# isabella232/kyverno

Hardware: AMD Instinct MI355X
Metric: resource×rule validate evals/sec (node) (higher is better)
Workload: dtype u8; 1 GPU; C2: synthetic Pods x 100 validate.pattern rules (image globs, ?*, quantities, |-lists); rules=100, pairs_per_gpu=100000000, output=full, parallelism=resource-shard x1, engine=specialized

## Files before the change

kyverno_amd/csrc/kvapi.cpp:

```cpp
#include <hip/hip_runtime.h>
#include <rccl/rccl.h>

#include <chrono>
#include <cstdio>
#include <cstring>

#define KVRT_DEVICE 1
#include "kvrt.hpp"
#include "kvdev.h"

namespace kvh {

struct DevPolicySet {
  DevBuf prog, preds, alts, conjs, atoms, rules, filters, kinds, strrefs, strpairs, sels, sellabels, selexprs, kgs,
      gsegs, gwords, pstr, fword, fbit, flist, frule, rcompact, gsdesc, gsmem;
  DevBuf view_dev;
  uint32_t gs_groups = 0, gs_members = 0;
  DevPS view{};
  std::vector<hipModule_t> mods;
  std::vector<hipFunction_t> fns;
  std::map<uint32_t, std::vector<hipFunction_t>> vfns;
  const std::vector<hipFunction_t>& fns_for(uint32_t full) const {
    auto it = vfns.find(full);
    return it == vfns.end() ? fns : it->second;
// ... 16 lines not shown
      }
    }
  }
};

struct DevBatchRes {
  DevBuf nodes, vals, res, kvs, bstr, nsbits, koff, klen, kstr, nsms, lsets, asets, tuprep, tupkent, kentrep, view_dev;
  DevBuf dpreds, dalts, dconjs, datoms, dgsegs, dgwords, dpstr, dps, dleaf, dynst;
  DevBuf pcol, pcold, pfam, perow;
  double pcol_ms = 0;
  DevBuf pre[5], dn[7], feg[2], fed[7], fe[5], fep[3], feacc, ferec, prest, dnst;
  double pre_ms = 0, deny_ms = 0, fe_ms = 0;
  DevBatch view{};
};
}

kv_policyset::kv_policyset() = default;
kv_policyset::~kv_policyset() = default;

namespace {

DevPolicySet& dev_ps(kv_policyset* s, int device) {
  std::lock_guard<std::mutex> g(s->mu);
  auto it = s->dev.find(device);
  if (it != s->dev.end()) return *it->second;
  auto d = std::make_unique<DevPolicySet>();
  const PolicySet& ps = s->ps;
  d->prog.upload(ps.prog, device);
  d->preds.upload(ps.preds, device);
  d->alts.upload(ps.alts, device);
  d->conjs.upload(ps.conjs, device);
  d->atoms.upload(ps.atoms, device);
  d->rules.upload(ps.rules, device);
  d->filters.upload(ps.filters, device);
  d->kinds.upload(ps.kinds, device);
  d->strrefs.upload(ps.strrefs, device);
  d->strpairs.upload(ps.strpairs, device);
  d->sels.upload(ps.selectors, device);
  d->sellabels.upload(ps.sellabels, device);
  d->selexprs.upload(ps.selexprs, device);
  d->kgs.upload(ps.kg_specs, device);
  d->gsegs.upload(ps.gsegs, device);
  d->gwords.upload(ps.gwords, device);
  d->pstr.upload_raw(ps.strs.data(), ps.strs.size(), device);
  DevPS& v = d->view;
  v.prog = (const Inst*)d->prog.p;
  v.preds = (const Pred*)d->preds.p;
  v.alts = (const Alt*)d->alts.p;
  v.conjs = (const Conj*)d->conjs.p;
  v.atoms = (const Atom*)d->atoms.p;
  v.rules = (const RuleRec*)d->rules.p;
  v.filters = (const MFilter*)d->filters.p;
  v.kinds = (const KindSpec*)d->kinds.p;
  v.strrefs = (const StrRef*)d->strrefs.p;
  v.strpairs = (const StrPair*)d->strpairs.p;
  v.sels = (const Selector*)d->sels.p;
  v.sellabels = (const SelLabel*)d->sellabels.p;
  v.selexprs = (const SelExpr*)d->selexprs.p;
  v.kg_specs = (const uint32_t*)d->kgs.p;
  v.gsegs = (const GSeg*)d->gsegs.p;
  v.gwords = (const GWord*)d->gwords.p;
  v.n_rules = (uint32_t)ps.rules.size();
  v.n_filters = (uint32_t)ps.filters.size();
  v.n_sels = (uint32_t)ps.selectors.size();
  v.pstr = (const uint8_t*)d->pstr.p;
  v.star_id = ps.lookup("*");
  if (v.star_id == KEY_NONE) v.star_id = KEY_NONE - 1;
  d->dev = device;
  if (s->jit) {
    const JitImage& J = *s->jit;
    std::map<std::string, hipFunction_t> byname;
    for (size_t i = 0; i < J.codes.size(); i++) {
      hipModule_t m;
      HIPCHK(hipModuleLoadData(&m, J.codes[i].data()));
      d->mods.push_back(m);
      hipFunction_t f;
      HIPCHK(hipModuleGetFunction(&f, m, J.kernel_name[i].c_str()));
      byname[J.kernel_name[i]] = f;
    }
    for (const JitImage::Variant& v : J.variants) {
      std::map<std::string, hipFunction_t> vname;
      for (size_t i = 0; i < v.codes.size() && i < J.kernel_name.size(); i++) {
        if (v.codes[i].empty()) continue;
        hipModule_t m;
        HIPCHK(hipModuleLoadData(&m, v.codes[i].data()));
        d->mods.push_back(m);
        hipFunction_t f;
        HIPCHK(hipModuleGetFunction(&f, m, J.kernel_name[i].c_str()));
        vname[J.kernel_name[i]] = f;
      }
      std::vector<hipFunction_t>& fv = d->vfns[v.full];
      for (auto& ch : J.chunks) {
        auto it = vname.find(ch.name);
        fv.push_back(it != vname.end() ? it->second : byname.at(ch.name));
      }
    }
    for (auto& ch : J.chunks) {
      auto it = byname.find(ch.name);
      if (it == byname.end()) throw std::runtime_error("specialized kernel " + ch.name + " missing");
      hipFunction_t f = it->second;
      d->fns.push_back(f);
      if (getenv("KVGPU_VERBOSE")) {
        int regs = 0, local = 0;
        (void)hipFuncGetAttribute(&regs, HIP_FUNC_ATTRIBUTE_NUM_REGS, f);
        (void)hipFuncGetAttribute(&local, HIP_FUNC_ATTRIBUTE_LOCAL_SIZE_BYTES, f);
        fprintf(stderr, "[kvgpu] %s: %zu rules, %d VGPRs, %d B scratch/lane\n", ch.name.c_str(), ch.rules.size(), regs,
                local);
      }
    }
    d->rcompact.upload(J.rec_compact, device);
    if (!J.gs_desc.empty()) {
      d->gs_groups = (uint32_t)(J.gs_desc.size() / 4u);
      d->gs_members = J.gs_members;
      d->gsdesc.upload(J.gs_desc, device);
      d->gsmem.upload(J.gs_mem, device);
    }
    if (J.mtup_words) {
      d->mtup_words = J.mtup_words;
      d->fac_slots = J.fac_slots;
      d->fword.upload(J.fac_word, device);
      d->fbit.upload(J.fac_bit, device);
      d->flist.upload(J.fac_flist, device);
      d->frule.upload(J.fac_rule, device);
      v.fac_word = (const uint32_t*)d->fword.p;
      v.fac_bit = (const uint32_t*)d->fbit.p;
      v.fac_flist = (const uint32_t*)d->flist.p;
      v.fac_rule = (const uint32_t*)d->frule.p;
      v.fac_slots = J.fac_slots;
      v.fac_words = J.mtup_words;
    }
    if (J.memo_words) {
      d->ptab_fn = byname.at("kvj_ptab");
      d->memo_words = J.memo_words;
      d->ptab_rows = (uint32_t)((J.memo_preds.size() + J.ptab_row - 1) / J.ptab_row);
    }
  }
  if (!ps.fpats.empty()) d->view_dev.upload_raw(&d->view, sizeof(DevPS), device);
  auto& ref = *d;
  s->dev[device] = std::move(d);
  return ref;
}

void build_pcol(const JitImage& J, const Batch& b, DevBatchRes* d, int device) {
  const auto t0 = std::chrono::steady_clock::now();
  const uint32_t nf = (uint32_t)J.fam_ncols.size(), j0 = J.fam_ncols.at(0);
  const uint64_t groups64 = (b.res.size() + KV_WG - 1) / KV_WG * (KV_WG / KV_LANES);
  if (groups64 > 0x3FFFFFFull) throw std::runtime_error("path columns: too many resources");
  const uint32_t groups = (uint32_t)groups64;
  d->pcold.upload(J.cols, device);
  d->perow.alloc((size_t)std::max<uint32_t>(1u, nf - 1) * (groups + 1) * sizeof(uint32_t), device);
  HIPCHK(hipMemset(d->perow.p, 0, d->perow.n));
  std::vector<ColFam> fams(nf);
  uint32_t n_wide = 0, n_narrow = 0;
  for (uint32_t f = 0; f < nf; f++) {
    fams[f].arr_col = J.fam_arr[f];
    fams[f].ncols = J.fam_ncols[f];
    fams[f].nw = J.fam_nw.at(f);
    fams[f].nb = J.fam_nb.at(f);
    fams[f].nn = J.fam_nn.at(f);
    fams[f].erow = f ? (uint32_t*)d->perow.p + (size_t)(f - 1) * (groups + 1) : nullptr;
    n_wide += fams[f].nw;
    n_narrow += fams[f].nn;
  }
  if (n_narrow && b.vals.size() + KV_PTAB_PSEUDO >= (1ull << KV_COL_PAYLOAD))
    throw std::runtime_error("path columns: more than 2^28 distinct values");
  d->pfam.upload(fams, device);
  const DevBatch* Bd = (const DevBatch*)d->view_dev.p;
  const ColDesc* cd = (const ColDesc*)d->pcold.p;
  std::vector<uint32_t> erow;
  if (nf > 1) {
    HIPCHK(launch_pcol_rows(Bd, cd, (const ColFam*)d->pfam.p, nf, groups, nullptr));
    erow.resize((size_t)(nf - 1) * (groups + 1));
    HIPCHK(hipMemcpy(erow.data(), d->perow.p, erow.size() * sizeof(uint32_t), hipMemcpyDeviceToHost));
  }
  auto row_words = [&](uint32_t f) { return (uint64_t)(3u * fams[f].nw + fams[f].nb + fams[f].nn) * KV_LANES; };
  const uint64_t root_words = (uint64_t)groups * row_words(0);
  uint64_t words = root_words;
  for (uint32_t f = 1; f < nf; f++) {
    fams[f].off_lo = (uint32_t)words;
    fams[f].off_hi = (uint32_t)(words >> 32);
    words += (uint64_t)erow[(size_t)(f - 1) * (groups + 1) + groups] * row_words(f);
  }
  if (words >= (1ull << 32)) throw std::runtime_error("path columns: more than 2^32 words");
  HIPCHK(hipMemcpy(d->pfam.p, fams.data(), fams.size() * sizeof(ColFam), hipMemcpyHostToDevice));
  d->pcol.alloc(std::max<uint64_t>(words, 1) * sizeof(uint32_t), device);
  uint32_t* pool = (uint32_t*)d->pcol.p;
  if (words > root_words) HIPCHK(hipMemset(pool + root_words, 0, (words - root_words) * sizeof(uint32_t)));
  HIPCHK(launch_pcol_build(Bd, cd, (const ColFam*)d->pfam.p, 0, j0, groups, false, pool, nullptr));
  HIPCHK(launch_pcol_build(Bd, cd, (const ColFam*)d->pfam.p, j0, (uint32_t)J.cols.size() - j0, groups, true, pool,
                           nullptr));
  HIPCHK(hipStreamSynchronize(nullptr));
  d->view.pcol = pool;
  d->pcol_ms = std::chrono::duration<double, std::milli>(std::chrono::steady_clock::now() - t0).count();
  if (getenv("KVGPU_VERBOSE"))
    fprintf(stderr,
            "[kvgpu] path columns: %u wide + %u narrow columns in %u families, %llu bytes (%.1f per resource), built in "
            "%.2f ms\n",
            n_wide, n_narrow, nf, (unsigned long long)(words * sizeof(uint32_t)),
            b.res.empty() ? 0.0 : (double)(words * sizeof(uint32_t)) / (double)b.res.size(), d->pcol_ms);
}

std::shared_ptr<DevBatchRes> dev_batch(kv_batch* bt, const PolicySet& ps, int device, const DevPS* pdev) {
  std::lock_guard<std::mutex> g(bt->mu);
  auto it = bt->dev.find(device);
  if (it != bt->dev.end()) return it->second;
  auto d = std::make_shared<DevBatchRes>();
  const Batch& b = bt->b;
  if (b.rmask.size() != b.n_rows || b.rwide.size() != b.n_rows || b.roff.size() != b.n_rows)
    throw std::runtime_error("batch: packed row arrays do not match the row count");
  hipStream_t us = StreamPool::get().take(device, hipStreamNonBlocking);
  DevBuf pc, rm, rw, ro;
  pc.upload_async(b.tcells, device, us);
  rm.upload_async(b.rmask, device, us);
  rw.upload_async(b.rwide, device, us);
  ro.upload_async(b.roff, device, us);
  d->vals.upload_async(b.vals, device, us);
  d->nodes.alloc(b.n_cells() * sizeof(Node), device);
  HIPCHK(launch_expand_rows((const uint64_t*)pc.p, (const uint64_t*)rm.p, (const uint64_t*)rw.p, (const uint32_t*)ro.p,
                            (const Val*)d->vals.p, b.n_rows, (Node*)d->nodes.p, us));
  d->res.upload_async(b.res, device, us);
  d->kvs.upload(b.kvs, device);
  d->bstr.upload_raw(b.strs.data(), b.strs.size(), device);
  d->nsbits.upload(b.ns_bits, device);
  std::vector<uint32_t> off, len;
  std::string ks;
  key_table(ps, b, &off, &len, &ks);
  d->koff.upload(off, device);
  d->klen.upload(len, device);
  d->kstr.upload_raw(ks.data(), ks.size(), device);
  d->nsms.upload(b.nsms, device);
  d->lsets.upload(b.lsets, device);
  d->asets.upload(b.asets, device);
  d->tuprep.upload(b.tup_rep, device);
  d->tupkent.upload(b.tup_kent, device);
  d->kentrep.upload(b.kent_rep, device);
  DevBatch& v = d->view;
  v.nodes = (const Node*)d->nodes.p;
  v.vals = (const Val*)d->vals.p;
  v.res = (const Res*)d->res.p;
  v.kvs = (const KV*)d->kvs.p;
  v.bstr = (const uint8_t*)d->bstr.p;
  v.ns_bits = (const uint32_t*)d->nsbits.p;
  v.key_off = (const uint32_t*)d->koff.p;
  v.key_len = (const uint32_t*)d->klen.p;
  v.kstr = (const uint8_t*)d->kstr.p;
  v.nsms = (const StrRef*)d->nsms.p;
  v.lsets = (const KVSet*)d->lsets.p;
  v.asets = (const KVSet*)d->asets.p;
  v.n_nsm = (uint32_t)b.nsms.size();
  v.n_lsets = (uint32_t)b.lsets.size();
  v.n_asets = (uint32_t)b.asets.size();
  v.ns_words = b.ns_words;
  v.n_res = (uint32_t)b.res.size();
  v.tup_rep = (const uint32_t*)d->tuprep.p;
  v.n_tup = (uint32_t)b.tup_rep.size();
  v.tup_kent = (const uint32_t*)d->tupkent.p;
  v.kent_rep = (const uint32_t*)d->kentrep.p;
  v.n_kent = (uint32_t)b.kent_rep.size();
  v.n_ns = (uint32_t)b.namespaces.size();
  {
    const DynHost& h = bt->dyn_host(ps);
    d->dpreds.upload(h.tbl.preds, device);
    d->dalts.upload(h.tbl.alts, device);
    d->dconjs.upload(h.tbl.conjs, device);
    d->datoms.upload(h.tbl.atoms, device);
    d->dgsegs.upload(h.tbl.gsegs, device);
    d->dgwords.upload(h.tbl.gwords, device);
    d->dpstr.upload_raw(h.tbl.strs.data(), h.tbl.strs.size(), device);
    DevPS dv{};
    dv.preds = (const Pred*)d->dpreds.p;
    dv.alts = (const Alt*)d->dalts.p;
    dv.conjs = (const Conj*)d->dconjs.p;
    dv.atoms = (const Atom*)d->datoms.p;
    dv.gsegs = (const GSeg*)d->dgsegs.p;
    dv.gwords = (const GWord*)d->dgwords.p;
    dv.pstr = (const uint8_t*)d->dpstr.p;
    d->dps.upload_raw(&dv, sizeof(DevPS), device);
    d->dleaf.upload(h.dleaf, device);
    d->dynst.upload(h.dyn_st, device);
    v.dps = (const DevPS*)d->dps.p;
    v.dleaf = (const uint32_t*)d->dleaf.p;
    v.dyn_st = (const uint8_t*)d->dynst.p;
  }
  auto up = [&](DevBuf* bufs, std::initializer_list<const std::vector<uint32_t>*> src, const uint32_t** dp) {
    for (const std::vector<uint32_t>* v : src) {
      bufs->alloc(std::max<size_t>(v->size() * sizeof(uint32_t), 16), device);
      if (!v->empty()) HIPCHK(hipMemcpyAsync(bufs->p, v->data(), v->size() * sizeof(uint32_t), hipMemcpyHostToDevice, us));
      *dp++ = (const uint32_t*)(bufs++)->p;
    }
  };
  auto up_blocks = [&](DevBuf* bufs, const CondHost& h, bool strict) {
    const uint32_t* dp[7] = {};
    up(bufs, {&h.sets, &h.ents, &h.outc, &h.truth, &h.unk}, dp);
    if (strict) up(bufs + 5, {&h.err, &h.oos}, dp + 5);
    return CondBlocks{dp[0], dp[1], dp[2], dp[3], dp[4], dp[5], dp[6], h.words};
  };
  struct Timed {
    hipEvent_t e0, e1;
    double* ms;
  };
  std::vector<Timed> timed;
  auto timed_launch = [&](double* ms, auto&& launch) {
    Timed t{nullptr, nullptr, ms};
    HIPCHK(hipEventCreate(&t.e0));
    HIPCHK(hipEventCreate(&t.e1));
    HIPCHK(hipEventRecord(t.e0, us));
    HIPCHK(launch());
    HIPCHK(hipEventRecord(t.e1, us));
    timed.push_back(t);
  };
  CondHost pre, dn;
  FeHost fh;
  CondBlocks pt{}, dt{};
  FeTables ft{};
  FePatTables qt{};
  DevBuf erec;
  const uint32_t n_sets = (uint32_t)ps.csets.size(), n_dsets = (uint32_t)ps.dsets.size(),
                 n_fsets = (uint32_t)ps.fsets.size(), n_pats = (uint32_t)ps.fpats.size();
  if (n_sets && !b.res.empty()) {
    build_pre(ps, b, &pre);
    pt = up_blocks(d->pre, pre, false);
    d->prest.alloc((size_t)n_sets * b.res.size(), device);
    v.pre_st = (const uint8_t*)d->prest.p;
  }
  if (n_dsets && !b.res.empty()) {
    build_deny(ps, b, &dn);
    dt = up_blocks(d->dn, dn, true);
  }
  if (n_fsets && !b.res.empty()) {
    build_foreach(ps, b, &fh);
    const uint32_t *dp[5], *gp[2];
    up(d->fe, {&fh.sets, &fh.lists}, dp);
    up(d->feg, {&fh.gate.sets, &fh.gate.ents}, gp);
    ft = fh.view();
    ft.gate = ft.deny = up_blocks(d->fed, fh.deny, true);
    ft.gate.sets = gp[0]; ft.gate.ents = gp[1];
    up(d->fe + 2, {&fh.el_res, &fh.el_ord, &fh.lstate}, dp + 2);
    ft.sets = dp[0]; ft.lists = dp[1]; ft.el_res = dp[2]; ft.el_ord = dp[3]; ft.lstate = dp[4];
    d->feacc.alloc((size_t)n_fsets * b.res.size() * sizeof(uint32_t), device);
    if (n_pats) {
      const uint32_t* qp[3];
      up(d->fep, {&fh.pats, &fh.chain, &fh.first}, qp);
      qt = FePatTables{qp[0], qp[1], qp[2], n_pats};
// ... 1276 lines not shown
```

kyverno_amd/csrc/kvcol.h:

```cpp
#pragma once

KV_FN Node col_step(const Node* __restrict__ N, const Node& n, uint32_t step, uint32_t* idx) {
  const Node z{0u, 0u, 0u, 0u};
  if (*idx == ABSENT || node_type(n.kt) != NT_MAP) {
    *idx = ABSENT;
    return z;
  }
  if (step & KV_COL_SCAN) {
    const uint32_t key = step & ~KV_COL_SCAN;
    for (uint32_t q = 0; q < n.b; q++) {
      const uint32_t c = ni(n.a + q);
      const Node t = N[c];
      if (node_key(t.kt) == key) {
        *idx = c;
        return t;
      }
    }
    *idx = ABSENT;
    return z;
  }
  if (step >= n.b) {
    *idx = ABSENT;
    return z;
  }
  const uint32_t c = ni(n.a + step);
  const Node t = N[c];
  if (node_type(t.kt) == NT_ABSENT) {
    *idx = ABSENT;
    return z;
  }
  *idx = c;
  return t;
}

KV_FN Node col_walk(const Node* __restrict__ N, uint32_t idx, const ColDesc& d, uint32_t* out) {
  Node n{0u, 0u, 0u, 0u};
  if (idx != ABSENT) n = N[idx];
  for (uint32_t s = 0; s < d.nsteps && s < KV_COL_MAXD; s++) n = col_step(N, n, d.steps[s], &idx);
  *out = idx;
  return n;
}

KV_FN Node col_cell(const Node& n, uint32_t idx, uint32_t arr_c) {
  if (idx == ABSENT) return Node{0u, 0u, 0u, 0u};
  const uint32_t t = node_type(n.kt);
  return Node{t | KV_COL_PRESENT, n.a, n.b, t == NT_MAP ? idx : t == NT_ARR ? arr_c : n.c};
}

KV_FN uint64_t col_fam_off(const ColFam& F) { return (uint64_t)F.off_lo | (uint64_t)F.off_hi << 32; }
KV_FN uint32_t col_row_words(const ColFam& F) { return (3u * F.nw + F.nb + F.nn) * KV_LANES; }

KV_FN void col_put(uint32_t* __restrict__ pool, uint64_t row, const ColFam& F, const ColDesc& d, uint32_t lane,
                   const Node& n, uint32_t idx) {
  if (d.fmt == KV_COLF_NARROW) {
    pool[row + (size_t)(3u * F.nw + F.nb + d.pos) * KV_LANES + lane] = kv_narrow_cell(n.kt, n.a, idx);
    return;
  }
  uint32_t* __restrict__ w = pool + row + (size_t)d.pos * (3u * KV_LANES) + 3u * lane;
  w[0] = n.kt;
  w[1] = n.a;
  w[2] = n.c;
  if (d.fmt == KV_COLF_WIDEB) pool[row + (size_t)(3u * F.nw + d.bpos) * KV_LANES + lane] = n.b;
}
KV_FN Node col_get(const uint32_t* __restrict__ pool, uint64_t row, const ColFam& F, const ColDesc& d, uint32_t lane) {
  const uint32_t* __restrict__ w = pool + row + (size_t)d.pos * (3u * KV_LANES) + 3u * lane;
  return Node{w[0], w[1], pool[row + (size_t)(3u * F.nw + d.bpos) * KV_LANES + lane], w[2]};
}

KV_FN uint32_t col_rows(const DevBatch& B, const ColDesc* cols, const ColFam* fams, uint32_t f, uint32_t r) {
  if (r >= B.n_res) return 0u;
  uint32_t idx;
  const Node n = col_walk(B.nodes, ni(B.res[r].root), cols[fams[f].arr_col], &idx);
  return idx != ABSENT && node_type(n.kt) == NT_ARR ? n.b : 0u;
}

KV_FN void col_build_root(const DevBatch& B, const ColDesc* cols, const ColFam* fams, uint32_t c, uint32_t r,
                          uint32_t* __restrict__ pool) {
  const ColDesc& d = cols[c];
  Node cell{0u, 0u, 0u, 0u};
  uint32_t idx = ABSENT;
  if (r < B.n_res) {
    const Node n = col_walk(B.nodes, ni(B.res[r].root), d, &idx);
    uint32_t arr_c = 0u;
    if (d.arr_fam) {
      const ColFam& F = fams[d.arr_fam];
      arr_c = (uint32_t)(col_fam_off(F) + (uint64_t)F.erow[r >> 6] * col_row_words(F));
    }
    cell = col_cell(n, idx, arr_c);
  }
  col_put(pool, (uint64_t)(r >> 6) * col_row_words(fams[0]), fams[0], d, r & (KV_LANES - 1), cell, idx);
}

KV_FN void col_build_elem(const DevBatch& B, const ColDesc* cols, const ColFam* fams, uint32_t c, uint32_t r,
                          uint32_t* __restrict__ pool) {
  const ColDesc& d = cols[c];
  const ColFam& F = fams[d.fam];
  const uint32_t lane = r & (KV_LANES - 1);
  const Node a = col_get(pool, (uint64_t)(r >> 6) * col_row_words(fams[0]), fams[0], cols[F.arr_col], lane);
  if (node_type(a.kt) != NT_ARR || a.kt == 0u) return;
  for (uint32_t i = 0; i < a.b; i++) {
    uint32_t idx;
    const Node n = col_walk(B.nodes, ni(a.a + i), d, &idx);
    col_put(pool, (uint64_t)a.c + (uint64_t)i * col_row_words(F), F, d, lane, col_cell(n, idx, 0u), idx);
  }
}
```

kyverno_amd/csrc/kvdev.h:

```cpp
#pragma once
#include <hip/hip_runtime.h>
#include <stdint.h>

#include "kvcell.h"
#include "kv_layout.h"
#include "kvdevtypes.h"

namespace kv {

hipError_t launch_validate(const DevPS* P, const DevBatch* B, uint32_t n_res, const DevOut& O, uint32_t rule_begin,
                           uint32_t rule_end, hipStream_t stream);

struct CondBlocks;
hipError_t launch_cond(bool strict, const CondBlocks& T, uint32_t n_res, uint32_t n_sets, uint8_t* st, hipStream_t stream);

struct FeTables;
struct FePatTables;
hipError_t launch_foreach(const FeTables& T, uint32_t n_res, uint32_t* fe_acc, uint8_t* fe_st, hipStream_t stream,
                          const FePatTables* Q = nullptr, const DevPS* P = nullptr, const DevBatch* B = nullptr,
                          uint2* erec = nullptr, uint2* fe_rec = nullptr);

hipError_t launch_mtab(const DevPS* P, const DevBatch* B, uint32_t words, uint32_t max_entities, uint32_t* ns,
                       uint32_t* an, uint32_t* sl, hipStream_t stream);

hipError_t launch_mfac(const DevPS* P, const DevBatch* B, uint32_t slots, uint32_t max_entities, uint32_t words,
                       uint32_t n_tup, uint32_t* mtup, hipStream_t stream);

hipError_t launch_gather_rows(const uint8_t* in, const uint32_t* inv, uint64_t n_rules, uint64_t n_res, uint8_t* out,
                              hipStream_t stream);

hipError_t launch_remap_u32(uint32_t* a, uint64_t n, const uint32_t* map, hipStream_t stream);

hipError_t launch_status_pack(const uint8_t* status, const uint8_t* sflag, uint32_t n_res, uint32_t n_rules,
                              const unsigned long long* cbase, uint32_t* ccnt, uint8_t* out, hipStream_t stream);

hipError_t launch_gsite_expand(const uint32_t* gsite, const uint32_t* gcnt, const GSiteDesc* desc, const uint32_t* mem,
                               uint32_t n_groups, uint32_t n_res, ErrRec8* err8, hipStream_t stream);
hipError_t launch_rec_compact(const uint8_t* status, const ErrRec8* err8, const ErrRec* errw, uint32_t n_res,
                              uint32_t n_rules, uint32_t* offs, unsigned long long* totals, unsigned long long* base,
                              ErrRec8* out8, ErrRec* outw, uint32_t* wide, int phase, const uint8_t* compact,
                              const uint32_t* order, unsigned long long* masks, const uint8_t* sflag, hipStream_t stream);

hipError_t launch_rec_codes(const ErrRec8* rec, const unsigned long long* base, uint32_t n_rules,
                            unsigned long long* tkey, uint8_t* code, uint32_t* raw, const unsigned long long* nbase,
                            ErrRec8* out, int phase, hipStream_t stream);

constexpr uint32_t KV_SCOPE_CHUNK = 65536;
constexpr uint32_t KV_SCOPE_LDS = 2048;

hipError_t launch_scope_totals(const unsigned long long* scounts, uint32_t n_scopes, uint32_t n_rules,
                               unsigned long long* counts, hipStream_t stream);
hipError_t launch_scope_counts(const uint8_t* status, const uint32_t* scope, uint32_t n_res, uint32_t n_rules,
                               uint32_t n_scopes, unsigned long long* out, hipStream_t stream);

hipError_t launch_expand_rows(const uint64_t* tcells, const uint64_t* rmask, const uint64_t* rwide, const uint32_t* roff,
                              const Val* vals, uint64_t n_rows, Node* nodes, hipStream_t stream);

hipError_t launch_pcol_rows(const DevBatch* B, const ColDesc* cols, const ColFam* fams, uint32_t n_fam,
                            uint32_t n_groups, hipStream_t stream);
hipError_t launch_pcol_build(const DevBatch* B, const ColDesc* cols, const ColFam* fams, uint32_t c0, uint32_t n,
                             uint32_t n_groups, bool elem, uint32_t* pool, hipStream_t stream);

}
```

kyverno_amd/csrc/kvdevtypes.h:

```cpp
#pragma once

namespace kv {

struct ErrRec {
  uint32_t kind_flags;
  uint32_t pnode;
  uint32_t keynode;
  uint32_t resnode;
  uint32_t idx[4];
};

struct ErrRec8 {
  uint32_t w0, w1;
};
constexpr uint32_t ERR8_WIDE = 1u << 6;
constexpr uint32_t ERR8_IDX_MASK = (1u << 26) - 1u;

struct DevPS {
  const Inst* prog;
  const Pred* preds;
  const Alt* alts;
  const Conj* conjs;
  const Atom* atoms;
  const RuleRec* rules;
  const MFilter* filters;
  const uint32_t* fflags;
  const KindSpec* kinds;
  const StrRef* strrefs;
  const StrPair* strpairs;
  const Selector* sels;
  const SelLabel* sellabels;
  const SelExpr* selexprs;
  const uint32_t* kg_specs;
  const GSeg* gsegs;
  const GWord* gwords;
  const uint8_t* pstr;
  uint32_t star_id;
  uint32_t n_rules;
  uint32_t n_filters, n_sels;
  const uint32_t* ptab;
  uint32_t n_vals;
  uint32_t mt_ns_words, mt_ann_words, mt_sel_words;
  const uint32_t* mt_ns;
  const uint32_t* mt_ann;
  const uint32_t* mt_sel;
  const uint32_t* mtup;
  uint32_t mtup_words;
  const uint32_t* mt_bitf;
  const uint32_t* fac_word;
  const uint32_t* fac_bit;
  const uint32_t* fac_flist;
  const uint32_t* fac_rule;
  uint32_t fac_slots, fac_words;
  uint32_t* fac_tab;
  uint64_t fac_off[5];
};
constexpr uint32_t KV_FAC_PRESENT = 0x80000000u;
constexpr uint32_t KV_FAC_MAXP = 8;
enum FacType : uint32_t { KV_FAC_KIND = 0, KV_FAC_NSM = 1, KV_FAC_ANN = 2, KV_FAC_SEL = 3, KV_FAC_NS = 4, KV_FAC_TYPES = 5 };

struct DevBatch {
  const Node* nodes;
  const Val* vals;
  const Res* res;
  const KV* kvs;
  const uint8_t* bstr;
  const uint32_t* ns_bits;
  const uint32_t* key_off;
  const uint32_t* key_len;
  const uint8_t* kstr;
  const StrRef* nsms;
  const KVSet* lsets;
  const KVSet* asets;
  uint32_t n_nsm, n_lsets, n_asets;
  uint32_t ns_words;
  uint32_t n_res;
  const uint32_t* tup_rep;
  uint32_t n_tup;
  const uint32_t* tup_kent;
  const uint32_t* kent_rep;
  uint32_t n_kent, n_ns;
  const DevPS* dps;
  const uint32_t* dleaf;
  const uint8_t* dyn_st;
  const uint32_t* pcol;
  const uint8_t* pre_st;
  const uint8_t* deny_st;
};

constexpr uint32_t KV_COL_MAXD = 12;
constexpr uint32_t KV_COL_SCAN = 0x80000000u;
constexpr uint32_t KV_COL_PRESENT = 16u;
constexpr uint32_t KV_COL_PAYLOAD = 28u;
enum ColFmt : uint32_t { KV_COLF_WIDE = 0, KV_COLF_WIDEB = 1, KV_COLF_NARROW = 2 };
struct ColDesc {
  uint32_t fam;
  uint32_t j;
  uint32_t nsteps;
  uint32_t arr_fam;
  uint32_t fmt;
  uint32_t pos;
  uint32_t bpos;
  uint32_t steps[KV_COL_MAXD];
};
struct ColFam {
  uint32_t arr_col, ncols;
  uint32_t nw, nb, nn;
  uint32_t off_lo, off_hi;
  uint32_t* erow;
};

struct DevOut {
  uint8_t* status;
  ErrRec8* err8;
  ErrRec* err;
  unsigned long long* counts;
  uint32_t full;
  unsigned long long* scounts;
  const uint32_t* scope;
  uint32_t* gsite;
  uint32_t* gcnt;
  uint8_t* sflag;
};

struct GSiteDesc {
  uint32_t n, gpre, moff, pad;
};

constexpr int KV_WG = 256;
constexpr int KV_RWG = 256;
constexpr uint32_t KV_RWAVES = (uint32_t)KV_RWG / 64u;
constexpr uint32_t KV_RSTRIDE = KV_RWG;
constexpr uint32_t KV_KROWS = 128u;
constexpr uint32_t KV_ROW0 = KV_RWAVES * KV_KROWS;
constexpr uint32_t KV_PTAB_PSEUDO = 3;
constexpr int KV_HIST = 8;

}
```

kyverno_amd/csrc/kvjit.hpp:

```cpp
#pragma once
#include <cstdint>
#include <map>
#include <string>
#include <vector>

#include "kvinternal.hpp"
#include "kvdevtypes.h"

namespace kvh {

struct JitChunk {
  std::vector<uint32_t> rules;
  std::string name;
};

struct JitKernelPlan {
  uint32_t first, count;
  int waves;
  std::vector<uint32_t> blocks;
  bool grouped = false;
};

struct JitImage {
  std::vector<JitKernelPlan> plan;
  std::string source;
  std::string common;
  std::vector<std::string> kernel_name, kernel_src;
  std::vector<std::vector<char>> codes;
  std::vector<JitChunk> chunks;
  std::vector<uint32_t> memo_preds;
  uint32_t memo_words = 0;
  uint32_t ptab_row = 1;
  uint32_t mtup_words = 0;
  std::vector<uint32_t> fac_word, fac_bit, fac_flist, fac_rule;
  uint32_t fac_slots = 0;
  std::vector<uint8_t> rec_compact;
  std::vector<uint32_t> gs_desc, gs_mem;
  uint32_t gs_members = 0;
  std::vector<kv::ColDesc> cols;
  std::vector<uint32_t> fam_arr, fam_ncols;
  std::vector<uint32_t> fam_nw, fam_nb, fam_nn;
  std::map<std::string, uint32_t> col_use;
  bool probe = false;
  double gen_ms = 0, compile_ms = 0;
  struct Variant {
    uint32_t full = 0;
    std::vector<std::vector<char>> codes;
  };
  std::vector<Variant> variants;
};

uint32_t jit_chunk_rules();
constexpr uint32_t kJitStamps = 16;
void jit_generate(const PolicySet& ps, uint32_t chunk_rules, JitImage* out);

void jit_build(const PolicySet& ps, JitImage* img);
uint64_t code_bytes(const JitImage& img);
struct RegVerdict {
  uint32_t priv, vgprs;
  bool calls;
  bool fits;
  bool scratch_ok;
  bool ships() const { return fits && scratch_ok; }
  bool probe_splits() const { return (priv != 0 && !calls) || !fits; }
};
RegVerdict reg_verdict_of(uint32_t priv, uint32_t vgprs, int waves, bool calls);
bool jit_plan_spills(JitImage* img, const std::vector<RegVerdict>& verdicts);
bool jit_load_plan(const std::string& key, JitImage* img);
void jit_save_plan(const std::string& key, const JitImage& img);

}
```

kyverno_amd/csrc/kvjitbuild.cpp:

```cpp
#include <hip/hiprtc.h>

#include <dlfcn.h>
#include <sched.h>
#include <spawn.h>
#include <sys/stat.h>
#include <sys/wait.h>

#include <cerrno>
#include <unistd.h>

#include <algorithm>
#include <atomic>
#include <chrono>
#include <cstdio>
#include <cstdlib>
#include <cstring>
#include <set>
#include <sstream>
#include <stdexcept>
#include <thread>

#include "kvjit.hpp"

extern char** environ;
// ... 116 lines not shown
        char* const argv[] = {&av[0][0], &av[1][0], &av[2][0], &av[3][0], nullptr};
        pid_t pid = 0;
        if (posix_spawn(&pid, jitc.c_str(), nullptr, nullptr, argv, environ) != 0) {
          errs[t] = "kvjit: cannot start " + jitc;
          return;
        }
        int status = 0;
        while (waitpid(pid, &status, 0) < 0 && errno == EINTR) continue;
        if (!WIFEXITED(status) || WEXITSTATUS(status) != 0 || !read_file(out, &img->codes[i])) {
          errs[t] = "kvjit: compiling " + img->kernel_name[i] + " failed (kvjitc status " + std::to_string(status) + ")";
          return;
        }
        unlink(src.c_str());
        unlink(out.c_str());
        const size_t d = ++done;
        if (progress) {
          const int64_t now =
              (int64_t)std::chrono::duration<double, std::milli>(std::chrono::steady_clock::now() - t0).count();
          int64_t prev = last_ms.load();
          if (now - prev >= 15000 && last_ms.compare_exchange_strong(prev, now))
            fprintf(stderr, "[kvgpu] hiprtc: %zu/%zu kernel programs compiled (%.0f s)\n", d, todo.size(), now / 1e3);
        }
      }
    });
  for (auto& x : th) x.join();
  rmdir(dir.c_str());
  for (auto& e : errs)
    if (!e.empty()) throw std::runtime_error(e);
}

bool co_kernel_info(const std::vector<char>& co, const std::string& name, uint32_t* private_seg, uint32_t* vgprs) {
  auto rd = [&](size_t off, size_t n, void* out) {
    if (off + n > co.size()) return false;
    memcpy(out, co.data() + off, n);
    return true;
  };
  if (co.size() < 64 || memcmp(co.data(), "\x7f" "ELF", 4) != 0 || co[4] != 2) return false;
  uint64_t shoff = 0;
  uint16_t shentsize = 0, shnum = 0;
  rd(0x28, 8, &shoff);
  rd(0x3A, 2, &shentsize);
  rd(0x3C, 2, &shnum);
  struct Sh { uint32_t name, type; uint64_t flags, addr, off, size; uint32_t link, info; uint64_t align, entsize; };
  std::vector<Sh> sh(shnum);
  for (uint16_t i = 0; i < shnum; i++)
    if (!rd(shoff + (uint64_t)i * shentsize, sizeof(Sh), &sh[i])) return false;
  bool kd = false, fn = false;
  for (const Sh& t : sh) {
    if (t.type != 2  || t.link >= shnum) continue;
    const Sh& strtab = sh[t.link];
    for (uint64_t o = t.off; o + 24 <= t.off + t.size; o += 24) {
      uint32_t nm = 0;
      uint16_t shndx = 0;
      uint64_t value = 0;
      rd(o, 4, &nm);
      rd(o + 6, 2, &shndx);
      rd(o + 8, 8, &value);
      if (strtab.off + nm >= co.size()) continue;
      const char* sn = co.data() + strtab.off + nm;
      const size_t maxlen = co.size() - (strtab.off + nm);
      const std::string sym(sn, strnlen(sn, maxlen));
      if (sym == name + ".kd" && shndx < shnum) {
        const Sh& sec = sh[shndx];
        kd = rd(sec.off + (value - sec.addr) + 4, 4, private_seg);
        uint32_t rsrc1 = 0;
        if (kd && rd(sec.off + (value - sec.addr) + 48, 4, &rsrc1)) *vgprs = ((rsrc1 & 0x3Fu) + 1u) * 8u;
      } else if (sym == name) {
        fn = true;
      }
    }
  }
  return kd && fn;
}

uint64_t common_hash(const std::string& common) {
  std::string opt_key;
  for (const char* o : kOpts) opt_key += std::string(o) + "\n";
  int hv = 0;
  (void)hiprtcVersion(&hv, &hv);
  opt_key += "hiprtc " + std::to_string(hv) + "\n";
  return fnv1a64(common, fnv1a64(opt_key));
}

std::string cache_file(const JitImage& img, size_t i, uint64_t hcommon) {
  char key[40];
  snprintf(key, sizeof key, "%016llx", (unsigned long long)fnv1a64(img.kernel_src[i], hcommon));
  return img.kernel_name[i] + "-" + key + ".co";
}

void jit_compile(JitImage* img) {
  auto t0 = std::chrono::steady_clock::now();
  const size_t K = img->kernel_src.size();
  img->codes.assign(K, {});
  const std::string dir = cache_dir();
  const uint64_t hcommon = common_hash(img->common);
  std::vector<std::string> paths(K);
  std::vector<size_t> todo;
  for (size_t i = 0; i < K; i++) {
    paths[i] = dir.empty() ? "" : dir + "/" + cache_file(*img, i, hcommon);
    if (paths[i].empty() || !read_file(paths[i], &img->codes[i])) todo.push_back(i);
  }
  unsigned T = std::min(16u, host_threads());
  if (const char* e = getenv("KVGPU_JIT_THREADS")) T = (unsigned)std::max(1, atoi(e));
  T = std::max(1u, std::min<unsigned>(T, (unsigned)todo.size()));
  const std::string jitc = jitc_path();
  const bool procs = !(getenv("KVGPU_JIT_PROCS") && getenv("KVGPU_JIT_PROCS")[0] == '0');
  if (!todo.empty() && procs && !jitc.empty() && todo.size() > 1) {
    compile_in_children(img, todo, jitc, T);
  } else {
    for (size_t i : todo) img->codes[i] = compile_one(img->common + img->kernel_src[i], img->kernel_name[i]);
  }
  if (!dir.empty())
    for (size_t i : todo) write_file_atomic(dir, paths[i], img->codes[i]);
  img->compile_ms += std::chrono::duration<double, std::milli>(std::chrono::steady_clock::now() - t0).count();
}

size_t program_of(const JitImage& img, const std::string& name) {
  return (size_t)(std::find(img.kernel_name.begin(), img.kernel_name.end(), name) - img.kernel_name.begin());
}

bool reg_verdict(const JitImage& img, size_t ci, int waves, RegVerdict* out) {
  uint32_t priv = 0, vgprs = 0;
  if (ci >= img.codes.size() || !co_kernel_info(img.codes[ci], img.kernel_name[ci], &priv, &vgprs)) return false;
  *out = reg_verdict_of(priv, vgprs, waves, img.kernel_src[ci].find("kv_dleaf_impl") != std::string::npos);
  return true;
}

std::string variant_common(const JitImage& img, uint32_t full) {
  return "#define KVJ_FULL " + std::to_string(full) + "u\n" + img.common;
}

}

RegVerdict reg_verdict_of(uint32_t priv, uint32_t vgprs, int waves, bool calls) {
  RegVerdict v{priv, vgprs, calls, false, false};
  v.fits = waves == 0 || vgprs <= 512u / (uint32_t)waves;
  v.scratch_ok = priv == 0 || (calls && waves == 0);
  return v;
}

bool jit_plan_spills(JitImage* img, const std::vector<RegVerdict>& verdicts) {
  std::vector<JitKernelPlan> next;
  bool changed = false;
  for (size_t k = 0; k < img->plan.size(); k++) {
    const JitKernelPlan& kp = img->plan[k];
    const RegVerdict& v = verdicts.at(k);
    if (v.ships()) {
      next.push_back(kp);
      continue;
    }
    changed = true;
    JitKernelPlan np = kp;
    const size_t big = (size_t)(std::max_element(np.blocks.begin(), np.blocks.end()) - np.blocks.begin());
    if (kp.grouped) {
      np.grouped = false;
    } else if (v.calls && v.fits) {
      np.waves = 0;
    } else if (kp.waves > 6 && np.blocks.size() > 1) {
      np.waves = kp.waves - 1;
    } else if (!np.blocks.empty() && np.blocks[big] > 1) {
      const uint32_t c = np.blocks[big], h = c / 2;
      np.blocks[big] = h;
      np.blocks.insert(np.blocks.begin() + big + 1, c - h);
    } else if (kp.waves > 1) {
      np.waves = kp.waves - 1;
    } else if (kp.waves == 1) {
      np.waves = 0;
    } else if (kp.count > 1) {
      const uint32_t h = kp.count / 2;
      next.push_back({kp.first, h, 0, std::vector<uint32_t>(h, 1u)});
      next.push_back({kp.first + h, kp.count - h, 0, std::vector<uint32_t>(kp.count - h, 1u)});
      continue;
    } else {
      throw std::runtime_error("kvjit: kernel " + img->chunks[k].name + " needs " + std::to_string(v.priv) +
                               " B of scratch per lane even without a launch bound");
    }
    next.push_back(np);
  }
  if (changed) img->plan = next;
  return changed;
}

namespace {

bool jit_plan_spills(JitImage* img) {
  std::vector<RegVerdict> verdicts(img->plan.size());
  for (size_t k = 0; k < img->plan.size(); k++)
    if (!reg_verdict(*img, program_of(*img, img->chunks[k].name), img->plan[k].waves, &verdicts[k]))
      throw std::runtime_error("kvjit: no kernel descriptor for " + img->chunks[k].name);
  return jit_plan_spills(img, verdicts);
}

void jit_compile_variants(JitImage* img) {
  img->variants.clear();
  for (uint32_t full : {3u, 8u}) {
    JitImage v;
    v.common = variant_common(*img, full);
    std::vector<size_t> at;
    for (size_t i = 0; i < img->kernel_name.size(); i++)
      if (img->kernel_name[i].rfind("kvj_r", 0) == 0) {
        v.kernel_name.push_back(img->kernel_name[i]);
        v.kernel_src.push_back(img->kernel_src[i]);
        at.push_back(i);
      }
    if (at.empty()) return;
    jit_compile(&v);
    img->compile_ms += v.compile_ms;
    JitImage::Variant out;
    out.full = full;
    out.codes.resize(img->kernel_name.size());
    for (size_t k = 0; k < img->chunks.size() && k < img->plan.size(); k++) {
      const size_t j = program_of(v, img->chunks[k].name);
      RegVerdict rv;
      if (reg_verdict(v, j, img->plan[k].waves, &rv) && rv.ships()) out.codes[at[j]] = std::move(v.codes[j]);
    }
    img->variants.push_back(std::move(out));
  }
}

void jit_refine_blocks(const PolicySet& ps, uint32_t chunk_rules, JitImage* img) {
  for (int round = 0; round < 12; round++) {
    JitImage probe;
    probe.probe = true;
    probe.col_use = img->col_use;
    std::vector<std::pair<size_t, size_t>> at;
    for (size_t k = 0; k < img->plan.size(); k++) {
      const JitKernelPlan& kp = img->plan[k];
      if (kp.blocks.size() < 2 || kp.waves == 0) continue;
      uint32_t first = kp.first;
      for (size_t b = 0; b < kp.blocks.size(); b++) {
        if (kp.blocks[b] > 1) {
          probe.plan.push_back({first, kp.blocks[b], kp.waves, {kp.blocks[b]}});
          at.push_back({k, b});
        }
        first += kp.blocks[b];
      }
    }
    if (probe.plan.empty()) return;
    jit_generate(ps, chunk_rules, &probe);
    jit_compile(&probe);
    img->compile_ms += probe.compile_ms;
    std::set<std::pair<size_t, size_t>> split;
    for (size_t i = 0; i < probe.plan.size(); i++) {
      const std::string& name = probe.chunks[i].name;
      RegVerdict v;
      if (!reg_verdict(probe, program_of(probe, name), probe.plan[i].waves, &v))
        throw std::runtime_error("kvjit: no kernel descriptor for probe " + name);
      if (v.probe_splits()) split.insert(at[i]);
    }
    if (split.empty()) return;
    for (size_t k = 0; k < img->plan.size(); k++) {
      std::vector<uint32_t> nb;
      for (size_t b = 0; b < img->plan[k].blocks.size(); b++) {
        const uint32_t c = img->plan[k].blocks[b];
        if (split.count({k, b})) nb.insert(nb.end(), {c / 2, c - c / 2});
        else nb.push_back(c);
      }
      img->plan[k].blocks = nb;
    }
  }
}

std::string jit_plan_key(const JitImage& img) {
  uint64_t h = common_hash(img.common);
  for (size_t i = 0; i < img.kernel_src.size(); i++) h = fnv1a64(img.kernel_src[i], fnv1a64(img.kernel_name[i], h));
  char key[40];
  snprintf(key, sizeof key, "%016llx", (unsigned long long)h);
  return key;
}

}

uint64_t code_bytes(const JitImage& img) {
  uint64_t n = 0;
  for (auto& c : img.codes) n += c.size();
  return n;
}

bool jit_load_plan(const std::string& key, JitImage* img) {
  const std::string dir = cache_dir();
  std::vector<char> text;
  if (dir.empty() || !read_file(dir + "/plan-" + key + ".txt", &text)) return false;
  std::vector<JitKernelPlan> plan;
  std::istringstream in(std::string(text.begin(), text.end()));
  for (std::string line; std::getline(in, line);) {
    if (line.rfind("kernel ", 0) != 0) continue;
    std::istringstream ls(line.substr(7));
    JitKernelPlan kp{0, 0, 0, {}};
    ls >> kp.first >> kp.count >> kp.waves >> kp.grouped;
    uint32_t sum = 0;
    for (uint32_t b; ls >> b; sum += b) kp.blocks.push_back(b);
    if (sum != kp.count || kp.blocks.empty()) return false;
    plan.push_back(kp);
  }
  if (plan.empty()) return false;
  img->plan = plan;
  return true;
}

void jit_save_plan(const std::string& key, const JitImage& img) {
  const std::string dir = cache_dir();
  if (dir.empty()) return;
  std::string t;
  for (const JitKernelPlan& kp : img.plan) {
    t += "kernel " + std::to_string(kp.first) + " " + std::to_string(kp.count) + " " + std::to_string(kp.waves) + " " +
         (kp.grouped ? "1" : "0");
    for (uint32_t b : kp.blocks) t += " " + std::to_string(b);
    t += "\n";
  }
  const uint64_t hc = common_hash(img.common);
  for (size_t i = 0; i < img.kernel_src.size(); i++) t += "co " + cache_file(img, i, hc) + "\n";
  for (const JitImage::Variant& v : img.variants) {
    const uint64_t hv = common_hash(variant_common(img, v.full));
    for (size_t i = 0; i < img.kernel_src.size(); i++)
      if (i < v.codes.size() && !v.codes[i].empty()) t += "co " + cache_file(img, i, hv) + "\n";
  }
  write_file_atomic(dir, dir + "/plan-" + key + ".txt", t);
}

static void jit_group_regions(const PolicySet& ps, uint32_t chunk, JitImage* img) {
  for (JitKernelPlan& kp : img->plan) kp.grouped = true;
  jit_generate(ps, chunk, img);
  jit_compile(img);
  bool back = false;
  for (size_t k = 0; k < img->plan.size(); k++) {
    RegVerdict v;
    if (!reg_verdict(*img, program_of(*img, img->chunks[k].name), img->plan[k].waves, &v))
      throw std::runtime_error("kvjit: no kernel descriptor for " + img->chunks[k].name);
    if (!v.ships()) {
      img->plan[k].grouped = false;
      back = true;
    }
  }
  if (!back) return;
  jit_generate(ps, chunk, img);
  jit_compile(img);
}

void jit_build(const PolicySet& ps, JitImage* img) {
  const uint32_t chunk = jit_chunk_rules();
  const char* dump = getenv("KVGPU_JIT_DUMP");
  jit_generate(ps, chunk, img);
  if (dump) write_file(dump, img->source);
  if (!getenv("KVGPU_JIT_SKIP_COMPILE")) {
    const std::string pkey = jit_plan_key(*img);
    const bool stored = jit_load_plan(pkey, img);
    if (!stored) {
      for (JitKernelPlan& kp : img->plan) kp.grouped = false;
      jit_refine_blocks(ps, chunk, img);
    }
    jit_generate(ps, chunk, img);
    bool settled = false;
    for (int round = 0; round < 64 && !settled; round++) {
      jit_compile(img);
      settled = !jit_plan_spills(img);
      if (!settled) jit_generate(ps, chunk, img);
    }
    if (!settled)
      throw std::runtime_error("kvjit: the register plan did not settle (kernels still spill after 64 re-plans)");
    if (!stored) jit_group_regions(ps, chunk, img);
    jit_compile_variants(img);
    jit_save_plan(pkey, *img);
    if (dump) write_file(dump, img->source);
  }
  if (const char* co = getenv("KVGPU_JIT_DUMP_CO")) {
    for (size_t i = 0; i < img->codes.size(); i++) write_file(std::string(co) + "." + img->kernel_name[i] + ".co", img->codes[i]);
    for (const JitImage::Variant& v : img->variants)
      for (size_t i = 0; i < v.codes.size(); i++)
        if (!v.codes[i].empty())
          write_file(std::string(co) + "." + img->kernel_name[i] + ".m" + std::to_string(v.full) + ".co", v.codes[i]);
  }
}

}
```

kyverno_amd/csrc/kvjitgen.cpp:

```cpp
#include <algorithm>
#include <chrono>
#include <cstdio>
#include <cstdlib>
#include <cstring>
#include <map>
#include <set>
#include <sstream>
#include <stdexcept>
#include <unordered_map>

#include "kvjit.hpp"
#include "kvdevtypes.h"

namespace kvh {

using namespace kv;

namespace {

const char* kPrelude =
#include "kvjit_prelude.inc"
    ;

std::string hex32(uint32_t v) {
  char b[16];
  snprintf(b, sizeof b, "0x%08xu", v);
  return b;
}
bool no_program(const RuleRec& rr) { return rr.route != 0 || rr.deny != 0; }
std::string u32(uint32_t v) { return std::to_string(v) + "u"; }
std::string u64(uint64_t v) { return std::to_string(v) + "ull"; }
std::string i64(int64_t v) {
  if (v == INT64_MIN) return "(-9223372036854775807ll - 1)";
  return std::to_string(v) + "ll";
}
std::string f64(double v) {
  uint64_t b;
  memcpy(&b, &v, 8);
  return "__longlong_as_double(" + i64((int64_t)b) + ")";
}

constexpr uint32_t kGslotMembers = 22u;

struct GenOpts {
  bool narrow, stamps, has_waves;
  int waves;
  uint32_t block_w;
  std::string diag;
  GenOpts() {
    const char* e = getenv("KVGPU_JIT_NARROW");
    narrow = !(e && e[0] == '0');
    stamps = getenv("KVGPU_JIT_STAMPS") != nullptr;
    e = getenv("KVGPU_JIT_WAVES");
    has_waves = e != nullptr;
    waves = e ? atoi(e) : 0;
    e = getenv("KVGPU_JIT_BLOCK_W");
    block_w = e && atoi(e) > 0 ? (uint32_t)atoi(e) : 0u;
    std::istringstream names((e = getenv("KVGPU_JIT_DIAG")) ? e : "");
    for (std::string t; std::getline(names, t, ',');)
      if (!t.empty()) diag += "#define KV_DIAG_" + t + " 1\n";
  }
};

struct Gen {
  struct Fam {
    std::string arr;
    std::map<std::string, uint32_t> idx;
    std::vector<std::vector<uint32_t>> steps;
    std::vector<uint32_t> use;
  };
  struct Form {
    std::string text;
    std::vector<uint32_t> preds, pns;
    std::vector<uint32_t> leafpcs;
  };

  const PolicySet& ps;
  const GenOpts opt;

  std::vector<uint32_t> mpreds;
  std::map<uint32_t, uint32_t> pslot;
  std::map<uint32_t, uint32_t> pmask;
  std::vector<Fam> fams;
  std::map<std::string, uint32_t> fam_of;
  std::map<std::string, uint32_t> use_seed;
  std::vector<uint32_t> gs_desc, gs_mem;
  uint32_t gs_members = 0;
  std::vector<uint32_t> mt_bits;
  std::vector<uint8_t> rec_slot;
  uint32_t gtab_n = 0;
  std::map<uint32_t, Form> forms;
  std::map<uint32_t, uint32_t> bslot;
  std::map<uint32_t, std::set<uint32_t>> glob_bytes;
  std::vector<std::pair<std::string, std::string>> helpers;
  std::set<uint32_t> globs_done, atoms_done, preds_done, blks_done;
  std::set<std::pair<char, uint32_t>> qglobs_done, qatoms_done, qpreds_done;
  bool dleaf_done = false;
  std::vector<std::pair<std::string, std::string>> kernels;

  struct Kern {
    uint32_t mt_kbase = 0;
    uint32_t gs0 = 0, gsn = 0;
    std::string decls;
    bool grouped = false;
  };

  explicit Gen(const PolicySet& p) : ps(p), rec_slot(p.rules.size(), 0) {
    fams.emplace_back();
    col_of(0, "R");
  }

  struct Helper : std::ostringstream {
    Gen& g;
    const std::string name;
    Helper(Gen& gg, std::string n) : g(gg), name(std::move(n)) {}
    ~Helper() { g.helpers.push_back({name, str()}); }
  };
  static std::string num(const char* prefix, uint32_t i) { return prefix + std::to_string(i); }

  enum ColUse : uint32_t { CU_WIDE = 1u, CU_B = 2u, CU_LEAF = 4u };
  void col_mark(int fam, uint32_t j, uint32_t use) {
    if (fam >= 0 && j != kNoCol) fams.at((size_t)fam).use.at(j) |= use;
  }
  static std::string col_macro(const char* what, uint32_t f, uint32_t j) {
    return std::string("KVC_") + what + "_" + std::to_string(f) + "_" + std::to_string(j);
  }
  static constexpr uint32_t kNoCol = 0xFFFFFFFFu;
  static bool expr_steps(const std::string& ex, std::vector<uint32_t>* out) {
    out->clear();
    size_t at = ex.find('/');
    while (at != std::string::npos) {
      const size_t nx = ex.find('/', at + 1);
      const std::string tok = ex.substr(at + 1, nx == std::string::npos ? std::string::npos : nx - at - 1);
      if (tok.size() < 2 || (tok[0] != 's' && tok[0] != 'k')) return false;
      const unsigned long v = strtoul(tok.c_str() + 1, nullptr, 10);
      if (v >= KV_COL_SCAN) return false;
      out->push_back((uint32_t)v | (tok[0] == 'k' ? KV_COL_SCAN : 0u));
      at = nx;
    }
    return out->size() <= KV_COL_MAXD;
  }
  uint32_t col_of(uint32_t f, const std::string& rel) {
    Fam& F = fams.at(f);
    auto it = F.idx.find(rel);
    if (it != F.idx.end()) return it->second;
    std::vector<uint32_t> st;
    if (!expr_steps(rel, &st)) return kNoCol;
    const uint32_t j = (uint32_t)F.steps.size();
    F.idx.emplace(rel, j);
    F.steps.push_back(st);
    F.use.push_back(0u);
    return j;
  }
  uint32_t family(const std::string& arr) {
    auto it = fam_of.find(arr);
    if (it != fam_of.end()) return it->second;
    if (col_of(0, arr) == kNoCol) return kNoCol;
    const uint32_t f = (uint32_t)fams.size();
    fams.emplace_back();
    fams.back().arr = arr;
    col_of(f, "");
    fam_of.emplace(arr, f);
    return f;
  }
  void col_plan(JitImage* out, std::string* defs) const {
    out->cols.clear();
    out->fam_arr.clear();
    out->fam_ncols.clear();
    out->fam_nw.clear();
    out->fam_nb.clear();
    out->fam_nn.clear();
    out->col_use.clear();
    std::ostringstream d;
    d << "#define KVC_LO_ROW(n, w) kv_leaf_word(P, N, n, w)\n"
      << "#define KVC_LW_ROW(n, w) kv_leaf_gather(P, n, w)\n"
      << "#define KVC_LA_ROW(n, w) kv_leaf_fix(P.ptab, P.n_vals, N, (n).a, (n).b, false, w)\n";
    for (uint32_t f = 0; f < fams.size(); f++) {
      const Fam& F = fams[f];
      out->fam_arr.push_back(f ? fams[0].idx.at(F.arr) : 0u);
      out->fam_ncols.push_back((uint32_t)F.steps.size());
      std::vector<uint32_t> use(F.steps.size(), 0u);
      for (const auto& kv : F.idx) {
        const std::string key = F.arr + "|" + kv.first;
        uint32_t u = F.use[kv.second];
        auto it = use_seed.find(key);
        if (it != use_seed.end()) u |= it->second;
        if (f == 0 && fam_of.count(kv.first)) u |= CU_WIDE | CU_B;
        use[kv.second] = u;
        out->col_use[key] = u;
      }
      uint32_t nw = 0, nb = 0, nn = 0;
      const size_t c0 = out->cols.size();
      for (uint32_t j = 0; j < F.steps.size(); j++) {
        ColDesc c{};
        c.fam = f;
        c.j = j;
        c.nsteps = (uint32_t)F.steps[j].size();
        for (uint32_t s = 0; s < c.nsteps; s++) c.steps[s] = F.steps[j][s];
        if (opt.narrow && !(use[j] & CU_WIDE)) {
          c.fmt = KV_COLF_NARROW;
          c.pos = nn++;
        } else {
          c.pos = nw++;
          c.fmt = KV_COLF_WIDE;
          if (use[j] & (CU_B | CU_LEAF)) {
            c.fmt = KV_COLF_WIDEB;
            c.bpos = nb++;
          }
        }
        out->cols.push_back(c);
      }
      out->fam_nw.push_back(nw);
      out->fam_nb.push_back(nb);
      out->fam_nn.push_back(nn);
      d << "#define KVC_W" << f << " " << (3u * nw + nb + nn) * KV_LANES << "u\n";
      for (uint32_t j = 0; j < F.steps.size(); j++) {
        const ColDesc& c = out->cols[c0 + j];
        d << "#define " << col_macro("LD", f, j) << "(b) ";
        if (c.fmt == KV_COLF_NARROW) {
          d << "kv_ldn(PC, (b) + " << u32((3u * nw + nb + c.pos) * KV_LANES) << " + ln_)\n"
            << "#define " << col_macro("IX", f, j) << "(n) (node_type((n).kt) == NT_MAP ? KV_NARROW_IDX : 0u)\n"
            << "#define " << col_macro("LO", f, j) << "(n, w) kv_leaf_word_n(P, N, n, w)\n"
            << "#define " << col_macro("LW", f, j) << "(n, w) kv_leaf_gather(P, n, w)\n"
            << "#define " << col_macro("LA", f, j) << "(n, w) kv_leaf_fix(P.ptab, P.n_vals, N, (n).a, 0u, true, w)\n";
        } else {
          if (c.fmt == KV_COLF_WIDEB)
            d << "kv_ldwb(PC, (b) + " << u32(c.pos * 3u * KV_LANES) << " + 3u * ln_, (b) + "
              << u32((3u * nw + c.bpos) * KV_LANES) << " + ln_)\n";
          else
            d << "kv_ldw(PC, (b) + " << u32(c.pos * 3u * KV_LANES) << " + 3u * ln_)\n";
          d << "#define " << col_macro("IX", f, j) << "(n) (node_type((n).kt) == NT_MAP ? (n).c : 0u)\n"
            << "#define " << col_macro("LO", f, j) << "(n, w) kv_leaf_word(P, N, n, w)\n"
            << "#define " << col_macro("LW", f, j) << "(n, w) kv_leaf_gather(P, n, w)\n"
            << "#define " << col_macro("LA", f, j) << "(n, w) kv_leaf_fix(P.ptab, P.n_vals, N, (n).a, (n).b, false, w)\n";
        }
      }
    }
    for (uint32_t f = 1; f < fams.size(); f++) out->cols.at(out->fam_arr[f]).arr_fam = f;
    *defs = d.str();
  }

  template <class Fn>
  void each_atom(uint32_t pi, Fn fn) const {
    const Pred& pr = ps.preds[pi];
    if (pr.kind != PK_STRING) return;
    for (uint32_t a = pr.first; a < pr.first + pr.count; a++)
      for (uint32_t c = ps.alts[a].first; c < ps.alts[a].first + ps.alts[a].count; c++) {
        fn(ps.conjs[c].a0);
        if (ps.conjs[c].kind != CJ_ATOM) fn(ps.conjs[c].a1);
      }
  }

  std::string seg_expr(const GSeg& sg, const std::string& k, bool aligned0) {
    const uint32_t nw = (sg.len + 3) / 4;
    std::ostringstream e;
    e << "([&]() -> bool { ";
    if (aligned0) {
      e << "uint32_t x = 0u; ";
      for (uint32_t i = 0; i < nw; i++) {
        const GWord& g = ps.gwords[sg.wfirst + i];
        if (g.mask == 0) continue;
        e << "x |= (base[" << i << "] ^ " << hex32(g.w) << ") & " << hex32(g.mask) << "; ";
      }
      e << "return x == 0u; })()";
      return e.str();
    }
    e << "const uint32_t k_ = " << k << ", a_ = k_ >> 2, sh_ = k_ & 3u; uint32_t lo_ = base[a_], hi_, x = 0u; ";
    for (uint32_t i = 0; i < nw; i++) {
      const GWord& g = ps.gwords[sg.wfirst + i];
      e << "hi_ = base[a_ + " << (i + 1) << "]; ";
      if (g.mask) e << "x |= (__builtin_amdgcn_alignbyte(hi_, lo_, sh_) ^ " << hex32(g.w) << ") & " << hex32(g.mask) << "; ";
      e << "lo_ = hi_; ";
    }
    e << "return x == 0u; })()";
    return e.str();
  }

  void glob_fn(uint32_t ai) {
    if (!globs_done.insert(ai).second) return;
    const Atom& A = ps.atoms[ai];
    Helper o(*this, num("g_glob_", ai));
    o << "__device__ __forceinline__ bool " << o.name
      << "(const uint8_t* __restrict__ s, uint32_t sl, bool ascii, const uint8_t* __restrict__ pstr) {\n";
    const uint32_t fl = A.gflags;
    if (fl & G_ALL) { o << "  return true;\n}\n"; return; }
    if (fl & G_EMPTY) { o << "  return sl == 0u;\n}\n"; return; }
    if (fl & G_HASQ)
      o << "  if (!ascii) return kv_glob(pstr + " << u32(A.s_off) << ", " << u32(A.s_len & 0x7FFFFFFFu) << ", s, sl);\n";
    o << "  if (sl < " << u32(A.gmin) << ") return false;\n";
    o << "  const uint32_t* __restrict__ base = (const uint32_t*)s;\n";
    const uint32_t n = A.gcount;
    const GSeg* segs = ps.gsegs.data() + A.gfirst;
    uint32_t i0 = 0, i1 = n;
    o << "  uint32_t pos = 0u, end = sl;\n";
    if (!(fl & G_LEAD)) {
      const GSeg& s0 = segs[0];
      if (n == 1 && !(fl & G_TRAIL)) {
        o << "  return sl == " << u32(s0.len) << " && " << seg_expr(s0, "0u", true) << ";\n}\n";
        return;
      }
      o << "  if (!" << seg_expr(s0, "0u", true) << ") return false;\n";
      o << "  pos = " << u32(s0.len) << ";\n";
      i0 = 1;
    }
    if (!(fl & G_TRAIL)) {
      const GSeg& st = segs[n - 1];
      o << "  if (end < pos + " << u32(st.len) << ") return false;\n";
      o << "  if (!" << seg_expr(st, "end - " + u32(st.len), false) << ") return false;\n";
      o << "  end -= " << u32(st.len) << ";\n";
      i1 = n - 1;
    }
    for (uint32_t i = i0; i < i1; i++) {
      const GSeg& sg = segs[i];
      const auto [j, cbyte] = seg_key(sg);
      if (j < 0) {
        o << "  { bool found = false;\n"
          << "    for (uint32_t k = pos; k + " << u32(sg.len) << " <= end; k++)\n"
          << "      if (" << seg_expr(sg, "k", false) << ") { pos = k + " << u32(sg.len) << "; found = true; break; }\n"
          << "    if (!found) return false; }\n";
        continue;
      }
      o << "  { if (end < pos + " << u32(sg.len) << ") return false;\n"
        << "    const uint32_t plo = pos + " << u32(j) << ", phi = end - " << u32(sg.len) << " + " << u32(j) << ";\n"
        << "    bool found = false;\n"
        << "    for (uint32_t wa = plo >> 2; wa <= (phi >> 2) && !found; wa++) {\n"
        << "      const uint32_t w = base[wa] ^ " << hex32(cbyte * 0x01010101u) << ";\n"
        << "      uint32_t m = (w - 0x01010101u) & ~w & 0x80808080u;\n"
        << "      while (m) {\n"
        << "        const uint32_t p = wa * 4u + ((uint32_t)__builtin_ctz(m) >> 3); m &= m - 1u;\n"
        << "        if (p < plo || p > phi) continue;\n"
        << "        const uint32_t k = p - " << u32(j) << ";\n"
        << "        if (" << seg_expr(sg, "k", false) << ") { pos = k + " << u32(sg.len) << "; found = true; break; }\n"
        << "      }\n"
        << "    }\n"
        << "    if (!found) return false; }\n";
    }
    o << "  (void)pos; (void)end;\n  return true;\n}\n";
  }

  static constexpr uint32_t kMaxBSlots = 48;
// ... 367 lines not shown
        << "    for (uint32_t i = 0; i < " << W << "u; i++) sw[i] = src[i < lastw ? i : lastw];\n"
        << "#pragma unroll\n"
        << "    for (uint32_t i = 0; i < " << W << "u; i++) lw[i] = sw[i];\n"
        << "    lw[" << W << "] = src[lastw];\n"
        << "    const uint32_t nwu_ = kv_wave_words(lastw, " << W << "u);\n";
      for (auto& [m, ks] : groups) {
        std::set<uint32_t> bytes;
        for (uint32_t k : ks) pred_bytes(mpreds[k], &bytes);
        o << "    if (vc & " << u32(m) << ") {\n";
        if (!bytes.empty()) {
          o << "      " << qv->mt << " bm[" << kMaxBSlots << "];\n";
          for (uint32_t c : bytes)
            o << "      bm[" << bslot.at(c) << "] = " << qv->bmk << "_n(sw, " << hex32(c * 0x01010101u) << ", nwu_);\n";
        } else {
          o << "      const " << qv->mt << "* bm = nullptr;\n";
        }
        for (const auto& [pi, wb] : pred_words(ks)) {
          o << "      { const bool p_ = " << qv->pfx << "_pred_" << pi << "(V, S, sw, lw, bm, pstr, type, n);";
          for (const auto& [wi, bits] : wb) o << " w[" << wi << "] |= p_ ? " << u32(bits) << " : 0u;";
          o << " }\n";
        }
        o << "    }\n";
      }
    }
    o << "  } else {\n";
    for (auto& [m, ks] : groups) {
      o << "    if (vc & " << u32(m) << ") {\n";
      for (const auto& [pi, wb] : pred_words(ks)) {
        o << "      if (g_pred_" << pi << "(V, S, E, pstr, type, n)) {";
        for (const auto& [wi, bits] : wb) o << " w[" << wi << "] |= " << u32(bits) << ";";
        o << " }\n";
      }
      o << "    }\n";
    }
    o << "  }\n  }\n";
    for (uint32_t i = 0; i < nw; i++) o << "  PT[(size_t)" << i << "u * NP + v] = w[" << i << "];\n";
    o << "}\n\n";
    kernels.push_back({"kvj_ptab", o.str()});
  }

  void dleaf_fn() {
    if (dleaf_done) return;
    dleaf_done = true;
    Helper o(*this, "g_dleaf_0");
    o << "__device__ __forceinline__ bool g_dleaf_0(const DevBatch& B, const Node* __restrict__ N, uint32_t dp, "
         "const Node& vn) { return kv_dleaf_impl(B, N, dp, vn); }\n"
      << "__device__ __noinline__ bool kv_dleaf_impl(const DevBatch& B, const Node* __restrict__ N, uint32_t dp, Node vn) {\n"
      << "  const uint32_t vt = node_type(vn.kt);\n"
      << "  if (vt == NT_ARR) {\n"
      << "    for (uint32_t k = 0; k < vn.b; k++) if (!pred_node(*B.dps, B, N, dp, ni(vn.a + k))) return false;\n"
      << "    return true;\n  }\n"
      << "  return pred_eval(*B.dps, B, dp, vt, vn);\n}\n";
  }

  void blk_fn(uint32_t f) {
    if (!blks_done.insert(f).second) return;
    const MFilter& F = ps.filters[f];
    for (uint32_t a : ps.filter_name_atoms.at(f)) glob_fn(a);
    Helper o(*this, num("g_blk_", f));
    o << "__device__ __forceinline__ bool " << o.name
      << "(const DevPS& P, const DevBatch& B, const Res* __restrict__ R, uint32_t rkind, uint32_t rflags) {\n"
      << "  if (sld(P.fflags + " << f << "u) & (MF_EMPTY | MF_UI_FAIL)) return false;\n";
    if (F.flags & MF_KINDS) {
      bool any_star = false;
      std::ostringstream k;
      k << "false";
      for (uint32_t i = F.kinds_first; i < F.kinds_first + F.kinds_count; i++) {
        const KindSpec& ks = ps.kinds[i];
        switch (ks.form) {
          case 3: any_star = true; break;
          case 0: k << " || rkind == " << u32(ks.kind); break;
          case 1: k << " || (rkind == " << u32(ks.kind) << " && R->version == " << u32(ks.version) << ")"; break;
          default:
            k << " || (R->group == " << u32(ks.group) << " && rkind == " << u32(ks.kind) << " && (R->version == "
              << u32(ks.version) << " || R->version == P.star_id))";
            break;
        }
      }
      if (!any_star) o << "  if (!(" << k.str() << ")) return false;\n";
    }
    const std::vector<uint32_t>& na = ps.filter_name_atoms.at(f);
    auto name_glob = [&](uint32_t a) {
      return "g_glob_" + std::to_string(a) + "(B.bstr + R->name_off, R->name_len, (rflags & RF_NAME_ASCII) != 0u, P.pstr)";
    };
    size_t k = 0;
    if (F.flags & MF_NAME) o << "  if (!" << name_glob(na.at(k++)) << ") return false;\n";
    if (F.flags & MF_NAMES) {
      o << "  if (!(false";
      for (; k < na.size(); k++) o << " || " << name_glob(na[k]);
      o << ")) return false;\n";
    }
    if (F.flags & MF_NSS) o << "  if (!mt_bit(P.mt_ns, " << u32(F.nss_bit) << ", B.n_nsm, R->nsm)) return false;\n";
    if (F.flags & MF_ANN) o << "  if (!mt_bit(P.mt_ann, " << u32(F.ann_bit) << ", B.n_asets, R->aset)) return false;\n";
    if (F.flags & MF_SEL) o << "  if (!mt_bit(P.mt_sel, " << u32(F.sel) << ", B.n_lsets, R->lset)) return false;\n";
    if (F.flags & MF_NSSEL)
      o << "  if (!(rflags & (RF_KIND_NAMESPACE | RF_KIND_EMPTY)) && !((B.ns_bits[R->ns_index * B.ns_words + "
        << (F.nssel_bit / 32) << "u] >> " << (F.nssel_bit % 32) << "u) & 1u)) return false;\n";
    o << "  return true;\n}\n";
  }

  void match_fn(uint32_t ri) {
    const RuleRec& rr = ps.rules[ri];
    for (uint32_t f = rr.m_first; f < rr.m_first + rr.m_count; f++) blk_fn(f);
    for (uint32_t f = rr.x_first; f < rr.x_first + rr.x_count; f++) blk_fn(f);
    auto call = [&](uint32_t f) { return "g_blk_" + std::to_string(f) + "(P, B, R, rkind, rflags)"; };
    auto combine = [&](uint32_t mode, uint32_t first, uint32_t count) {
      std::ostringstream e;
      if (mode == 0 || count == 0) {
        e << call(first);
      } else {
        e << "(";
        for (uint32_t f = first; f < first + count; f++) e << (f > first ? (mode == 1 ? " || " : " && ") : "") << call(f);
        e << ")";
      }
      return e.str();
    };
    Helper o(*this, num("g_match_", ri));
    o << "__device__ __forceinline__ bool " << o.name
      << "(const DevPS& P, const DevBatch& B, const Res* __restrict__ R, uint32_t rkind, uint32_t rflags) {\n"
      << "  if (!" << combine(rr.m_mode, rr.m_first, rr.m_count) << ") return false;\n"
      << "  return !" << combine(rr.x_mode, rr.x_first, rr.x_count) << ";\n}\n";
  }

  static uint32_t prog_end(const PolicySet& ps, uint32_t pc) {
    while ((ps.prog[pc].op & 0xFF) != OP_DONE) pc++;
    return pc;
  }

  static constexpr uint32_t FIN = 0x7F000000u, ACT = 0x80000000u;

  struct HVar {
    std::string idx, node;
    int fam = -1;
    uint32_t j = kNoCol;
  };
  struct HWord {
    std::string var;
    HVar hv;
    uint32_t word = 0;
  };
  struct HoistTable {
    std::string prefix;
    std::map<std::string, HVar> vars;
    std::vector<std::string> cells;
    std::vector<HWord> words;
    std::vector<char> order;
    std::set<std::string> have;
    size_t cflushed = 0, wflushed = 0, oflushed = 0;
    void add_cell(const std::string& c) { cells.push_back(c); order.push_back('c'); }
    void add_word(const HWord& w) { words.push_back(w); order.push_back('w'); }
    uint32_t n = 0;
    int fam = -1;
    std::string troot, cell0;
    std::string flush(bool grouped) {
      std::string s;
      if (!grouped) {
        for (; oflushed < order.size(); oflushed++) {
          if (order[oflushed] == 'c') {
            s += cells[cflushed++];
            continue;
          }
          const HWord& x = words[wflushed++];
          s += "  const uint32_t " + x.var + " = " +
               (x.hv.fam >= 0 ? col_macro("LO", (uint32_t)x.hv.fam, x.hv.j) : std::string("KVC_LO_ROW")) + "(" + x.hv.node +
               ", " + std::to_string(x.word) + "u);\n";
        }
        return s;
      }
      oflushed = order.size();
      for (; cflushed < cells.size(); cflushed++) s += cells[cflushed];
      if (wflushed == words.size()) return s;
      std::vector<std::string> nodes;
      std::string fix;
      for (size_t i = wflushed; i < words.size(); i++) {
        const HWord& x = words[i];
        const bool col = x.hv.fam >= 0;
        const std::string args = "(" + x.hv.node + ", " + std::to_string(x.word) + "u);\n";
        s += "  uint32_t " + x.var + " = " + (col ? col_macro("LW", (uint32_t)x.hv.fam, x.hv.j) : std::string("KVC_LW_ROW")) + args;
        if (std::find(nodes.begin(), nodes.end(), x.hv.node) == nodes.end()) nodes.push_back(x.hv.node);
        fix += "    if (node_type(" + x.hv.node + ".kt) == NT_ARR) " + x.var + " = " +
               (col ? col_macro("LA", (uint32_t)x.hv.fam, x.hv.j) : std::string("KVC_LA_ROW")) + args;
      }
      wflushed = words.size();
      s += "  if (__ballot(";
      for (size_t i = 0; i < nodes.size(); i++) s += (i ? " || " : "") + ("node_type(" + nodes[i] + ".kt) == NT_ARR");
      return s + ") != 0ull) {  // some leaf cell is an array (rare)\n" + fix + "  }\n";
    }
  };

  struct RGen {
    uint32_t ri = 0, b = 0, e = 0, maxd = 1;
    std::vector<std::pair<uint32_t, uint32_t>> loops;
    std::vector<std::string> expr;
    std::vector<HVar> hv;
    std::vector<std::vector<std::pair<int, uint32_t>>> csrc;
    std::set<uint32_t> resume;
    std::set<uint32_t> carry_ok, carry_err;
    std::vector<char> lean, post_alt;
    std::vector<uint32_t> post_flags, skip_to;
    uint32_t q = 0;
    bool uses_anchor = false, uses_keyglob = false;
    bool grp = false;
    uint32_t gn = 1, grow = 0, gsri = 0, gspn = 0;
    std::vector<uint32_t> gri, gdpn;
    std::map<uint32_t, uint32_t> gslot;
    std::string gtab;
    bool gsite = false;
    uint32_t gl = 0, gpre = 0;
    uint32_t max_level = 0;
    std::string s;
  };

  HVar hoist(HoistTable& T, const std::string& pexpr, const HVar& p, uint32_t a, uint32_t aux) {
    const bool scan = (aux & AUX_SCAN) != 0;
    const std::string ex = pexpr + (scan ? "/k" : "/s") + std::to_string(a);
    auto it = T.vars.find(ex);
    if (it != T.vars.end()) return it->second;
    HVar h{T.prefix + "h" + std::to_string(T.n), T.prefix + "hn" + std::to_string(T.n)};
    T.n++;
    std::ostringstream c;
    const uint32_t j = T.fam >= 0 ? col_of((uint32_t)T.fam, T.fam == 0 ? ex : ex.substr(T.troot.size())) : kNoCol;
    if (j != kNoCol) {
      h.fam = T.fam;
      h.j = j;
      c << "  const Node " << h.node << " = " << col_macro("LD", (uint32_t)T.fam, j) << "(" << T.cell0 << ");\n"
        << "  const uint32_t " << h.idx << " = " << h.node << ".kt == 0u ? ABSENT : "
        << col_macro("IX", (uint32_t)T.fam, j) << "(" << h.node << ");\n";
      T.add_cell(c.str());
      T.vars.emplace(ex, h);
      return h;
    }
    col_mark(p.fam, p.j, CU_WIDE | CU_B);
    c << "  uint32_t " << h.idx << " = ABSENT; Node " << h.node << "{0u, 0u, 0u, 0u};\n";
    if (scan) {
      c << "  if (node_type(" << p.node << ".kt) == NT_MAP) for (uint32_t q_ = 0u; q_ < " << p.node << ".b; q_++) { "
        << "const uint32_t c_ = ni(" << p.node << ".a + q_); const Node t_ = N[c_]; if (node_key(t_.kt) == " << u32(a)
        << ") { " << h.idx << " = c_; " << h.node << " = t_; break; } }\n";
    } else {
      c << "  { const bool ok_ = node_type(" << p.node << ".kt) == NT_MAP && " << u32(a) << " < " << p.node << ".b; "
        << "const uint32_t c_ = ok_ ? ni(" << p.node << ".a + " << u32(a) << ") : 0u; const Node t_ = N[c_]; "
        << "const bool hit_ = ok_ && node_type(t_.kt) != NT_ABSENT; const uint32_t m_ = hit_ ? 0x07060504u : 0x0c0c0c0cu; "
        << h.idx << " = hit_ ? c_ : ABSENT; " << h.node << " = Node{__builtin_amdgcn_perm(t_.kt, 0u, m_), "
        << "__builtin_amdgcn_perm(t_.a, 0u, m_), __builtin_amdgcn_perm(t_.b, 0u, m_), __builtin_amdgcn_perm(t_.c, 0u, m_)}; }\n";
    }
    T.add_cell(c.str());
    T.vars.emplace(ex, h);
    return h;
  }

  struct Region {
    int kind = 0;
    uint32_t rb = 0, re = 0;
    uint32_t jre = 0;
    std::string se;
    std::set<uint32_t>*jumps = nullptr, *err_jumps = nullptr;
    std::string li0;
    HoistTable* T = nullptr;
    std::string troot;
  };

  struct GInfo {
    std::vector<uint32_t> members, pns0, leafpcs;
    std::vector<uint32_t> dpn;
    std::vector<std::vector<uint32_t>> preds;
  };

  struct Block {
    Kern& kern;
    const uint32_t hbase;
    std::vector<uint32_t> rules;
    std::vector<GInfo> ginfo;
    std::map<uint32_t, size_t> gof;
    std::vector<RGen> gs;
    HoistTable global;
    size_t K = 0;
    Block(Kern& k, uint32_t hb) : kern(k), hbase(hb) {
      global.prefix = "g";
      global.fam = 0;
      global.cell0 = "gw_";
    }
    uint32_t mask_words() const { return ((uint32_t)rules.size() + 31) / 32; }
    const RGen* at(uint32_t q) const {
      for (const RGen& x : gs)
        if (x.q == q) return &x;
      return nullptr;
    }
    const GInfo* group_of(uint32_t ri, bool* member) const {
      auto it = gof.find(ri);
      *member = it != gof.end() && ginfo[it->second].members[0] != ri;
      return it == gof.end() ? nullptr : &ginfo[it->second];
    }
  };

  void emit_region(Block& B, RGen& g, const Region& R, std::ostream& w) {
    const std::string& s = g.s;
    auto C = [&](uint32_t d) { return "c" + std::to_string(d) + s; };
    auto L = [&](uint32_t pc) { return "R" + std::to_string(g.ri) + "_L" + std::to_string(pc); };
    auto jump = [&](uint32_t t, bool err = false) -> std::string {
      if (t >= R.rb && t < R.jre) return "goto " + L(t) + ";";
      if (R.kind == 0 && t >= R.jre) {
        g.resume.insert(t);
        (err ? R.err_jumps : R.jumps)->insert(t);
        return "{ rs" + s + " = " + u32(t) + "; goto " + R.se + "; }";
      }
      throw std::runtime_error("kvjit: jump out of a fused region (rule " + std::to_string(g.ri) + ")");
    };
    auto finish = [&](const std::string& st) {
      if (R.kind != 0) throw std::runtime_error("kvjit: rule end inside a fused loop");
      return "{ rs" + s + " = FIN_ | " + st + "; goto " + R.se + "; }";
    };
    auto li = [&](uint32_t lv) { return lv == 0 && R.kind == 1 ? R.li0 : "li" + std::to_string(lv) + s; };
    const bool G = g.grp;
    const std::string al = "al" + s;
    auto gdone = [&]() -> std::string {
      if (R.kind == 0) return "{ rs" + s + " = FIN_ | ST_STORED_; goto " + R.se + "; }";
      return "goto " + L(R.re) + ";";
    };
    auto gfin = [&](const std::string& m, uint32_t kind, uint32_t pn, uint32_t catch_pc) {
      const PostChain pcn = post_chain(g, catch_pc);
      if (!pcn.pure || pcn.alt) throw std::runtime_error("kvjit: impure error chain in rule group");
      std::string st;
      if (kind == E_CPU) st = "ST_CPU";
      else if (pcn.flags & (EF_COND | EF_GLOBAL)) st = "ST_SKIP";
      else {
        st = kind == E_LEN ? "ST_ERROR" : "ST_FAIL";
        if (g.uses_anchor) st = "((areg" + s + " & ~apres" + s + ") ? ST_ERROR : " + st + ")";
      }
      std::ostringstream r;
      r << "kv_gfin<" << (g.gtab.empty() ? "false" : "true") << ", " << (g.gsite ? "true" : "false")
        << ">(O, n_res, r, valid, " << m << ", " << st << ", " << u32(kind | (pcn.flags << 4) | (pn << 8));
      for (uint32_t lv = 0; lv < 4; lv++) r << ", " << (lv <= g.max_level ? li(lv) : std::string("0u"));
      r << ", s_w + " << u32(KV_ROW0 + g.grow * KV_RSTRIDE) << ", " << u32(g.grow) << ", " << (g.gtab.empty() ? std::string("nullptr") : g.gtab) << ", "
        << u32(g.gn) << ", " << u32(g.gri[0]) << ", " << u32(g.gsri) << ", " << u32(g.gspn) << ", "
        << (!g.gsite && g.gn >= kGslotMembers ? "true" : "false");
      if (g.gsite) r << ", s_gc_ + " << u32(KV_RWAVES * g.gl) << ", " << u32(g.gpre);
      r << ");";
      return r.str();
    };
    auto raise = [&](uint32_t kind, uint32_t pn, uint32_t catch_pc) {
      if (pn >= (1u << 24)) throw std::runtime_error("kvjit: pattern node id exceeds 24 bits");
      if (G) return "{ " + gfin(al, kind, pn, catch_pc) + " " + al + " = 0u; " + gdone() + " }";
      std::ostringstream r;
      r << "{ ek" << s << " = " << u32(kind) << " | " << u32(pn << 8) << ";";
      for (uint32_t lv = 0; lv <= g.max_level && lv < 4; lv++) r << " ei" << lv << s << " = " << li(lv) << ";";
      if (g.uses_keyglob) r << " ekn" << s << " = kn" << s << ";";
      r << " " << jump(catch_pc, true) << " }";
      return r.str();
    };
    auto known = [&](uint32_t d) {
      if (d >= g.expr.size() || g.expr[d].empty()) return false;
      const std::string& ex = g.expr[d];
      return ex[0] == 'R' || (R.T && ex.compare(0, R.troot.size(), R.troot) == 0);
    };
    auto IDX = [&](uint32_t d) {
      if (d < g.csrc.size())
        for (const auto& cj : g.csrc[d]) col_mark(cj.first, cj.second, CU_WIDE);
    };
    auto NODE = [&](uint32_t d, uint32_t use = 0u) -> std::string {
      if (known(d)) {
        col_mark(g.hv[d].fam, g.hv[d].j, use);
        return g.hv[d].node;
      }
      IDX(d);
      return "N[" + C(d) + "]";
    };
    auto table_for = [&](uint32_t d) -> HoistTable* {
      const std::string& ex = g.expr[d];
      if (ex[0] == 'R') return &B.global;
      if (R.T && ex.compare(0, R.troot.size(), R.troot) == 0) return R.T;
      return nullptr;
    };
    auto absent_or = [&](uint32_t d, const char* cmp) {
      const std::string test = "node_type(" + NODE(d) + ".kt) " + cmp;
      return known(d) ? test : C(d) + " == ABSENT || " + test;
    };
    auto set_unknown = [&](uint32_t from) {
      for (uint32_t x = from; x < g.expr.size(); x++) g.expr[x].clear();
    };
    auto lookup = [&](uint32_t d, uint32_t a, uint32_t aux, bool assign) -> std::string {
      const uint32_t laux = aux & AUX_SCAN;
      HoistTable* T = known(d) ? table_for(d) : nullptr;
      if (T) {
        HVar h = hoist(*T, g.expr[d], g.hv[d], a, laux);
        if (assign) {
          set_unknown(d + 1);
          g.expr[d + 1] = g.expr[d] + (laux ? "/k" : "/s") + std::to_string(a);
          g.hv[d + 1] = h;
          if (h.fam >= 0) g.csrc.at(d + 1).push_back({h.fam, h.j});
        }
        return h.idx;
      }
      if (assign) set_unknown(d + 1);
      IDX(d);
      return "lookup_op(N, " + C(d) + ", " + u32(a) + ", " + u32(laux) + ")";
    };
    const std::string ek = "ek" + s;
    const std::string kindof = "(" + ek + " & 15u)";
    const std::string alt_reset =
        "  " + ek + " = 0u;" + (g.uses_anchor ? " areg" + s + " = 0ull; apres" + s + " = 0ull;" : "") + "\n";
    auto next_elem = [&](const std::string& lv, const std::string& cur, uint32_t body) {
      return "  if (li" + lv + s + " + 1u < ll" + lv + s + ") { li" + lv + s + "++; " + cur + " = ni(lf" + lv + s + " + li" + lv +
             s + "); " + jump(body) + " }\n";
    };

    for (uint32_t pc = R.rb; pc < R.re; pc++) {
      const Inst& in = ps.prog[pc];
      const uint32_t op = in.op & 0xFF, d = (in.op >> 8) & 0xFF, aux = (in.op >> 16) & 0xFF;
      const std::string cd = C(d), cn = C(d + 1);
      const uint32_t lv = aux & 3;
      const std::string L_lv = std::to_string(lv);
      w << L(pc) << ":;\n";
      switch (op) {
        case OP_MAPCHK:
          w << "  if (" << absent_or(d, "!= NT_MAP") << ") " << raise(E_TYPE_MAP, in.a, in.c) << "\n";
          break;
        case OP_ARRCHK:
          w << "  if (" << absent_or(d, "!= NT_ARR") << ") " << raise(E_TYPE_ARR, in.a, in.c) << "\n";
          break;
        case OP_AREG: {
          const std::string bit = "(1ull << " + std::to_string(aux & 63) + ")";
          w << "  areg" << s << " |= " << bit << "; if (" << lookup(d, in.a, aux, false) << " != ABSENT) apres" << s
            << " |= " << bit << ";\n";
          break;
        }
        case OP_KEY:
          w << "  " << cn << " = " << lookup(d, in.a, aux, true) << "; if (" << cn << " == ABSENT) " << jump(in.b) << "\n";
          break;
        case OP_KEYV:
          w << "  " << cn << " = " << lookup(d, in.a, aux, true) << ";\n";
          break;
        case OP_KEYGLOB:
          if (G) throw std::runtime_error("kvjit: KEYGLOB in a rule group");
          set_unknown(d + 1);
          IDX(d);
          w << "  { uint32_t nd_; if (!keyglob_op(P, B, N, " << cd << ", " << u32(in.op) << ", " << u32(in.a) << ", "
            << u32(in.c) << ", &nd_, &kn" << s << ")) " << jump(in.b) << " " << cn << " = nd_; }\n";
          break;
        case OP_SCOPE_END:
          if (G) break;
          if (in.c == 0) w << "  if (" << kindof << ") " << ek << " |= " << u32(aux << 4) << ";\n";
          else w << "  if (" << kindof << ") { " << ek << " |= " << u32(aux << 4) << "; " << jump(in.c, true) << " }\n";
          break;
        case OP_POS_END:
          if (G) throw std::runtime_error("kvjit: POS_END in a rule group");
          w << "  if (" << kindof << ") { if (" << ek << " & " << u32(EF_COND << 4) << ") " << ek << " = 0u; else "
            << jump(in.c, true) << " }\n";
          break;
        case OP_NEG:
          w << "  if (" << lookup(d, in.a, aux, false) << " != ABSENT) " << raise(E_NEG, in.b, in.c) << "\n";
          break;
        case OP_STAR:
          w << "  if (" << absent_or(d + 1, "== NT_NULL") << ") " << raise(E_STAR, in.b, in.c) << "\n";
          break;
        case OP_LEAF: {
          const uint32_t slot = G ? g.gslot.at(pc) : slot_for(in.a);
          const uint32_t word = slot / 32;
          HoistTable* T = known(d) ? table_for(d) : nullptr;
          std::string wx;
          if (T) {
            const HVar& hvd = g.hv[d];
            const std::string hn = hvd.node;
            wx = hn + "_w" + std::to_string(word);
            col_mark(hvd.fam, hvd.j, CU_LEAF);
            if (T->have.insert(wx).second) T->add_word(HWord{wx, hvd, word});
          } else {
            IDX(d);
            wx = "kv_leaf_word(P, N, (" + cd + " != ABSENT ? N[" + cd + "] : Node{0u, 0u, 0u, 0u}), " + u32(word) + ")";
          }
          if (G) {
            const uint32_t mask = g.gn >= 32 ? 0xFFFFFFFFu : (1u << g.gn) - 1u;
            w << "  { const uint32_t f_ = " << al << " & ~((" << wx << " >> " << u32(slot % 32) << ") & " << hex32(mask)
              << ");\n    if (f_) { " << gfin("f_", E_VALUE, in.b, in.c) << " " << al << " &= ~f_; if (!" << al << ") "
              << gdone() << " } }\n";
          } else {
            w << "  if (!(((" << wx << " >> " << u32(slot % 32) << ") & 1u) != 0u)) " << raise(E_VALUE, in.b, in.c) << "\n";
          }
          break;
        }
        case OP_VLEAF:
          if (G) throw std::runtime_error("kvjit: VLEAF in a rule group");
          if (known(d)) w << "  { const Node vn_ = " << NODE(d, CU_WIDE | CU_B) << ";\n";
          else {
            IDX(d);
            w << "  { Node vn_{0u, 0u, 0u, 0u}; if (" << cd << " != ABSENT) vn_ = N[" << cd << "];\n";
          }
          dleaf_fn();
          w << "    if (!g_dleaf_0(B, N, B.dleaf[(size_t)" << u32(in.a) << " * n_res + r], vn_)) "
            << raise(E_VALUE, in.b, in.c) << " }\n";
          break;
        case OP_RAISE:
          w << "  " << raise(in.b, in.a, in.c) << "\n";
          break;
        case OP_EXISTCHK:
          w << "  if (" << absent_or(d, "!= NT_ARR") << ") " << raise(E_EXIST_RESTYPE, in.a, in.c) << "\n";
          break;
        case OP_LENCHK:
          w << "  if (" << NODE(d, CU_WIDE | CU_B) << ".b < " << u32(in.a) << ") " << raise(E_LEN, in.b, in.c) << "\n";
          break;
        case OP_INDEX:
          w << "  " << cn << " = ni(" << NODE(d, CU_WIDE) << ".a + " << u32(in.a) << ");\n";
          set_unknown(d + 1);
          break;
        case OP_LOOP_BEGIN:
          if (R.kind == 0 && lv == 0) {
            set_unknown(d + 1);
            w << "  { rs" << s << " = " << u32(in.a + 1) << " | ACT_; goto " << R.se << "; }\n";
            break;
          }
          [[fallthrough]];
        case OP_EXIST_BEGIN:
          if (G && op == OP_EXIST_BEGIN) throw std::runtime_error("kvjit: EXIST in a rule group");
          set_unknown(d + 1);
          w << "  { const Node an_ = " << NODE(d, CU_WIDE | CU_B) << "; lf" << L_lv << s << " = an_.a; ll" << L_lv << s << " = an_.b; li"
            << L_lv << s << " = 0u;\n    if (an_.b == 0u) ";
          if (op == OP_LOOP_BEGIN) w << jump(in.a + 1);
          else w << raise(E_EXIST_FAIL, in.b, in.c);
          w << "\n    " << cn << " = ni(an_.a); }\n";
          break;
        case OP_LOOP_END:
          if (!G)
            w << "  if (" << kindof << ") { if (" << ek << " & " << u32(EF_COND << 4) << ") " << ek << " = 0u; else "
              << jump(in.c, true) << " }\n";
          w << next_elem(L_lv, cn, in.a + 1);
          set_unknown(d + 1);
          break;
        case OP_EXIST_END:
          if (G) throw std::runtime_error("kvjit: EXIST in a rule group");
          w << "  if (!" << kindof << ") " << jump(pc + 1) << "\n  " << ek << " = 0u;\n"
            << next_elem(L_lv, cn, in.a + 1) << "  " << raise(E_EXIST_FAIL, in.b, in.c) << "\n";
          set_unknown(d + 1);
          break;
        case OP_ALT_BEGIN:
          if (G) throw std::runtime_error("kvjit: anyPattern in a rule group");
          w << alt_reset;
          break;
        case OP_ALT_END:
          if (G) throw std::runtime_error("kvjit: anyPattern in a rule group");
          w << "  if (" << kindof << " == 0u) " << finish("ST_PASS") << "\n  if (" << kindof << " == E_CPU) "
            << finish("ST_CPU") << "\n";
          if (in.b) w << "  " << finish("ST_FAIL") << "\n";
          else w << alt_reset;
          break;
        case OP_DONE:
          if (R.kind != 0) throw std::runtime_error("kvjit: rule end inside a fused loop");
          if (G) {
            w << "  { rs" << s << " = FIN_ | ST_PASS; goto " << R.se << "; }\n";
            break;
          }
          w << "  { const uint32_t k_ = " << kindof << ";\n    rs" << s << " = FIN_ | (k_ == 0u ? ST_PASS : k_ == E_CPU ? ST_CPU : ("
            << ek << " & " << u32((EF_COND | EF_GLOBAL) << 4) << ") ? ST_SKIP : ";
          if (g.uses_anchor) w << "(areg" << s << " & ~apres" << s << ") ? ST_ERROR : ";
          w << "k_ == E_LEN ? ST_ERROR : ST_FAIL);\n    goto " << R.se << "; }\n";
          break;
        default:
          break;
      }
    }
  }

  RGen analyze(uint32_t ri) {
    RGen g;
    g.ri = ri;
    g.s = "_" + std::to_string(ri);
    g.b = ps.rules[ri].prog;
    g.e = prog_end(ps, g.b);
    int nest = 0;
    for (uint32_t pc = g.b; pc <= g.e; pc++) {
      const Inst& in = ps.prog[pc];
      const uint32_t op = in.op & 0xFF, d = (in.op >> 8) & 0xFF, aux = (in.op >> 16) & 0xFF;
      g.maxd = std::max(g.maxd, d + 2);
      if (op == OP_AREG) g.uses_anchor = true;
      if (op == OP_KEYGLOB) g.uses_keyglob = true;
      if (op == OP_LOOP_BEGIN || op == OP_EXIST_BEGIN) {
        if (op == OP_LOOP_BEGIN && nest == 0 && (aux & 3) == 0) g.loops.push_back({pc, in.a});
        g.max_level = std::max(g.max_level, aux & 3);
        nest++;
      } else if (op == OP_LOOP_END || op == OP_EXIST_END) {
        nest--;
      }
    }
    g.expr.assign(g.maxd + 1, "");
    g.hv.assign(g.maxd + 1, HVar{});
    g.csrc.assign(g.maxd + 2, {});
    g.expr[0] = "R";
    g.hv[0] = HVar{"root", "rootn", 0, 0u};
    return g;
  }

  struct PostChain {
    bool pure = false, alt = false;
    uint32_t flags = 0;
  };
  PostChain post_chain(const RGen& g, uint32_t pc, bool cond = false) const {
    PostChain r;
    for (int steps = 0; steps < 100000 && pc >= g.b && pc <= g.e; steps++) {
      const Inst& in = ps.prog[pc];
      const uint32_t op = in.op & 0xFF, aux = (in.op >> 16) & 0xFF;
      switch (op) {
        case OP_SCOPE_END:
          r.flags |= aux;
          cond |= (aux & EF_COND) != 0;
          pc = in.c ? in.c : pc + 1;
          continue;
        case OP_POS_END:
        case OP_LOOP_END:
          if (cond) return r;
          pc = in.c;
          continue;
        case OP_NOP:
        case OP_METACHK:
          pc++;
          continue;
        case OP_DONE:
          r.pure = true;
          return r;
        case OP_ALT_END:
          if (in.b) r.pure = r.alt = true;
          return r;
        default:
          return r;
      }
    }
    return r;
  }

  std::string done_status(const RGen& g, const std::string& ekx, bool alt) const {
    std::ostringstream w;
    const std::string k = "(" + ekx + " & 15u)";
    if (alt) {
      w << "(" << k << " == 0u ? ST_PASS : " << k << " == E_CPU ? ST_CPU : ST_FAIL)";
      return w.str();
    }
    w << "(" << k << " == 0u ? ST_PASS : " << k << " == E_CPU ? ST_CPU : (" << ekx << " & "
      << u32((EF_COND | EF_GLOBAL) << 4) << ") ? ST_SKIP : ";
    if (g.uses_anchor) w << "(areg" << g.s << " & ~apres" << g.s << ") ? ST_ERROR : ";
    w << k << " == E_LEN ? ST_ERROR : ST_FAIL)";
    return w.str();
  }

  const Form& form_of(uint32_t ri) {
    const auto [it, fresh] = forms.try_emplace(ri);
    if (fresh) group_form(ri, &it->second);
    return it->second;
  }
  void group_form(uint32_t ri, Form* F) const {
    const RuleRec& rr = ps.rules[ri];
    if (rr.route != 0 || rr.dyn || rr.pre || rr.deny) return;
    const uint32_t b = rr.prog, e = prog_end(ps, b);
    std::ostringstream f;
    auto rel = [&](uint32_t t) { return (int64_t)t - (int64_t)b; };
    for (uint32_t pc = b; pc <= e; pc++) {
      const Inst& in = ps.prog[pc];
      const uint32_t op = in.op & 0xFF, aux = (in.op >> 16) & 0xFF;
      f << (in.op & 0xFFFFFFu) << ':';
      switch (op) {
        case OP_MAPCHK:
        case OP_ARRCHK: F->pns.push_back(in.a); f << rel(in.c); break;
        case OP_AREG:
        case OP_KEYV:
        case OP_INDEX: f << in.a; break;
        case OP_KEY: f << in.a << ',' << rel(in.b); break;
        case OP_SCOPE_END:
          if (aux & EF_COND) return;
          f << (in.c ? rel(in.c) : -1);
          break;
        case OP_NEG: f << in.a << ','; F->pns.push_back(in.b); f << rel(in.c); break;
        case OP_STAR: F->pns.push_back(in.b); f << rel(in.c); break;
        case OP_LEAF:
          F->preds.push_back(in.a);
          F->leafpcs.push_back(pc - b);
          F->pns.push_back(in.b);
          f << rel(in.c);
          break;
        case OP_RAISE: f << in.b << ','; F->pns.push_back(in.a); f << rel(in.c); break;
        case OP_LENCHK: f << in.a << ','; F->pns.push_back(in.b); f << rel(in.c); break;
        case OP_LOOP_BEGIN: f << rel(in.a); break;
        case OP_LOOP_END: f << rel(in.a) << ',' << rel(in.c); break;
        case OP_DONE:
        case OP_NOP:
        case OP_METACHK: break;
        default: return;
      }
      f << ';';
    }
    F->text = f.str();
  }

  bool name_dependent(uint32_t ri) const {
    const RuleRec& rr = ps.rules[ri];
    for (uint32_t f = rr.m_first; f < rr.m_first + rr.m_count; f++)
      if (ps.filters[f].flags & (MF_NAME | MF_NAMES)) return true;
    for (uint32_t f = rr.x_first; f < rr.x_first + rr.x_count; f++)
      if (ps.filters[f].flags & (MF_NAME | MF_NAMES)) return true;
    return false;
  }
  std::string mt_cond(const Kern& kn, uint32_t ri, uint32_t row) const {
    const uint32_t p = kn.mt_kbase * 32u + row;
    std::string c = "((mw" + std::to_string(p / 32u) + " >> " + std::to_string(p % 32u) + "u) & 1u)";
    if (name_dependent(ri)) c += " && g_match_" + std::to_string(ri) + "(P, B, R, rkind, rflags)";
    return c;
  }


  void form_groups(const std::vector<uint32_t>& rules_in, Block* B) {
    std::map<std::string, size_t> open;
    for (uint32_t ri : rules_in) {
      const Form& F = form_of(ri);
      if (F.text.empty()) continue;
      auto it = open.find(F.text);
      if (it != open.end()) {
// ... 309 lines not shown
    emit_region(B, g, R, w);
    const Inst& end = ps.prog[le];
    if (end.c <= le) throw std::runtime_error("kvjit: loop exit target inside the loop");
    const bool lean = g.lean[k];
    const std::string ek = "ek" + g.s, rs = "rs" + g.s, am = mword("am", k, g.q), bit = mbit(g.q);
    out << "    if (" << (lean ? am + " & " + bit : rs + " & ACT_") << ") {\n";
    if (lean && !g.grp) out << "      " << clear_err(g) << "\n";
    out << "      c" << (d + 1) << g.s << " = el" << L.tag << ";\n" << w.str() << "R" << g.ri << "_L" << le << ":;\n";
    if (g.grp) {
      out << "      if (!al" << g.s << ") " << (lean ? am + " &= ~" + bit : rs + " = FIN_ | ST_STORED_") << ";\n";
    } else {
      out << "      if (" << ek << " & 15u) { if (" << ek << " & " << u32(EF_COND << 4) << ") " << ek << " = 0u; else ";
      if (lean) {
        const std::string ekx = g.post_flags[k] ? "(" + ek + " | " + u32(g.post_flags[k] << 4) + ")" : ek;
        out << "{\n        " << am << " &= ~" << bit << ";\n"
            << "  " << store_st(B, g.q, &g, done_status(g, ekx, g.post_alt[k]), ekx) << "      } }\n";
      } else {
        out << rs << " = " << u32(end.c) << "; }\n";
        g.resume.insert(end.c);
      }
    }
    out << "    }\n";
    g.resume.insert(le + 1);
    for (uint32_t x = d + 1; x < g.expr.size(); x++) g.expr[x].clear();
  }

  void emit_fused_loop(Block& B, size_t k, const std::string& key, const std::vector<RGen*>& grp, const std::string& tag,
                       std::ostream& body) {
    const RGen& g0 = *grp[0];
    const uint32_t d0 = (ps.prog[g0.loops[k].first].op >> 8) & 0xFF;
    const std::string arr_node = key[0] == 'U' ? "N[c" + std::to_string(d0) + g0.s + "]" : g0.hv[d0].node;
    if (key[0] == 'U') {
      for (const auto& cj : g0.csrc.at(d0)) col_mark(cj.first, cj.second, CU_WIDE);
    } else {
      col_mark(g0.hv[d0].fam, g0.hv[d0].j, CU_WIDE | CU_B);
    }
    Loop L;
    L.k = k;
    L.tag = tag;
    L.troot = "E" + tag;
    L.T.prefix = "l" + tag + "_";
    L.fam = key[0] == 'R' && fams[0].idx.count(key) ? family(key) : kNoCol;
    if (L.fam != kNoCol) {
      L.T.fam = (int)L.fam;
      L.T.troot = L.troot;
      L.T.cell0 = "ec" + tag;
    }
    std::ostringstream bodies;
    for (RGen* gp : grp) loop_body(B, *gp, L, bodies);
    std::vector<uint32_t> gmask(B.mask_words(), 0);
    for (const RGen* gp : grp)
      if (gp->lean[k]) gmask[gp->q / 32] |= 1u << (gp->q % 32);
    body << "  { // fused loop " << tag << " over " << key << " (" << grp.size() << " rules)\n"
         << "    uint32_t fn" << tag << " = 0u, ff" << tag << " = 0u, fe" << tag << " = 0u;\n    if (((0u";
    for (const RGen* gp : grp)
      if (!gp->lean[k]) body << " | rs" << gp->s;
    body << ") & ACT_)";
    for (uint32_t w = 0; w < gmask.size(); w++)
      if (gmask[w]) body << " | (am" << k << "_" << w << " & " << u32(gmask[w]) << ")";
    body << ") { const Node an_ = " << arr_node << "; ff" << tag << " = an_.a; fn" << tag << " = an_.b; fe" << tag
         << " = an_.c; }\n";
    body << "    for (uint32_t fli" << tag << " = 0u; fli" << tag << " < fn" << tag << "; fli" << tag << "++) {\n"
         << "      const uint32_t el" << tag << " = ni(ff" << tag << " + fli" << tag << ");\n";
    if (L.fam != kNoCol)
      body << "      const uint32_t ec" << tag << " = fe" << tag << " + fli" << tag << " * KVC_W" << L.fam
           << ";\n      const Node eln" << tag << " = " << col_macro("LD", L.fam, 0) << "(ec" << tag << ");\n";
    else
      body << "      const Node eln" << tag << " = N[el" << tag << "];\n";
    body << L.T.flush(B.kern.grouped) << bodies.str() << "    }\n";
    for (const RGen* gp : grp)
      if (!gp->lean[k]) body << "    rs" << gp->s << " &= ~ACT_;\n";
    body << "  }\n";
  }

  void emit_fused_loops(Block& B, size_t k, std::ostream& body) {
    std::map<std::string, std::vector<RGen*>> groups;
    std::vector<std::string> order;
    for (RGen& g : B.gs) {
      if (k >= g.loops.size()) continue;
      const uint32_t d = (ps.prog[g.loops[k].first].op >> 8) & 0xFF;
      const std::string key = g.expr[d].empty() ? "U" + std::to_string(g.ri) : g.expr[d];
      if (!groups.count(key)) order.push_back(key);
      groups[key].push_back(&g);
    }
    uint32_t li = 0;
    for (const std::string& key : order) emit_fused_loop(B, k, key, groups[key], std::to_string(k) + "_" + std::to_string(li++), body);
  }

  void emit_rule_state(const Block& B, std::ostream& k) const {
    for (uint32_t ri : B.rules)
      if (!B.gof.count(ri)) k << "  uint32_t rs_" << ri << " = FIN_ | ST_NOMATCH;\n";
    for (const RGen& g : B.gs) {
      const std::string& s = g.s;
      if (g.grp) k << "  uint32_t rs" << s << " = FIN_ | ST_STORED_, al" << s << " = 0u;\n";
      k << "  uint32_t ek" << s << " = 0u";
      for (uint32_t lv = 0; lv <= g.max_level && lv < 4; lv++) k << ", ei" << lv << s << " = 0u";
      if (g.uses_keyglob) k << ", kn" << s << " = ABSENT, ekn" << s << " = ABSENT";
      k << ";\n";
      if (g.uses_anchor) k << "  uint64_t areg" << s << " = 0ull, apres" << s << " = 0ull;\n";
      k << "  uint32_t c0" << s << " = root";
      for (uint32_t d = 1; d < g.maxd; d++) k << ", c" << d << s << " = ABSENT";
      k << ";\n";
      k << "  uint32_t";
      for (uint32_t l = 0; l <= g.max_level && l < 4; l++)
        k << (l ? "," : "") << " li" << l << s << " = 0u, lf" << l << s << " = 0u, ll" << l << s << " = 0u";
      k << ";\n";
    }
  }

  static void check_resumes(const Block& B) {
    for (const RGen& g : B.gs)
      for (uint32_t t : g.resume) {
        bool ok = false;
        for (size_t k = 0; k <= g.loops.size() && !ok; k++) ok = t >= segment(g, k).first && t < segment(g, k).second;
        if (!ok) throw std::runtime_error("kvjit: resume target " + std::to_string(t) + " of rule " +
                                         std::to_string(g.ri) + " is not in a segment");
      }
  }

  std::string fused_block(Kern& kern, const std::vector<uint32_t>& rules_in, uint32_t hbase, std::vector<uint32_t>* order) {
    Block B(kern, hbase);
    form_groups(rules_in, &B);
    *order = B.rules;
    prepare_rules(&B);
    std::ostringstream body;
    for (size_t k = 0; k <= B.K; k++) {
      std::ostringstream seg;
      for (RGen& g : B.gs)
        if (k <= g.loops.size()) emit_segment(B, g, k, seg);
      if (k < B.K) {
        body << "  uint32_t";
        for (uint32_t w = 0; w < B.mask_words(); w++)
          body << (w ? "," : "") << " am" << k << "_" << w << " = 0u, sk" << k << "_" << w << " = 0u";
        body << ";\n";
      }
      body << B.global.flush(B.kern.grouped) << seg.str();
      if (k < B.K) emit_fused_loops(B, k, body);
    }
    check_resumes(B);
    std::ostringstream k;
    emit_rule_state(B, k);
    for (uint32_t q = 0; q < B.rules.size(); q++)
      if (no_program(ps.rules[B.rules[q]])) k << match_code(B, q) << store(B, q);
    k << body.str();
    return k.str();
  }

  static uint32_t kernel_lds(uint32_t nr) { return KV_ROW0 + nr * KV_RSTRIDE; }
  static int lds_waves(uint32_t nr) {
    const uint32_t g = 1280u, b = (kernel_lds(nr) + g - 1u) / g * g;
    return (int)std::max<uint32_t>(1u, (160u * 1024u) / std::max(b, g) * KV_RWAVES / 4u);
  }
  std::vector<uint32_t> group_kernel(const std::string& name, const std::vector<std::vector<uint32_t>>& chs, int waves,
                                     bool grouped) {
    std::vector<std::string> blocks;
    std::vector<std::pair<uint32_t, uint32_t>> rows;
    std::vector<uint32_t> rules;
    uint32_t nr_all = 0;
    for (const auto& c : chs) nr_all += (uint32_t)c.size();
    if (nr_all > KV_KROWS) throw std::runtime_error("kvjit: at most KV_KROWS rules per kernel (KVGPU_JIT_CHUNK)");
    Kern kern;
    kern.mt_kbase = (uint32_t)(mt_bits.size() / 32u);
    kern.gs0 = (uint32_t)(gs_desc.size() / 4u);
    kern.grouped = grouped;
    for (const auto& c : chs) {
      std::vector<uint32_t> ord;
      rows.push_back({(uint32_t)rules.size(), (uint32_t)c.size()});
      blocks.push_back(fused_block(kern, c, (uint32_t)rules.size(), &ord));
      rules.insert(rules.end(), ord.begin(), ord.end());
    }
    mt_bits.insert(mt_bits.end(), rules.begin(), rules.end());
    while (mt_bits.size() % 32u) mt_bits.push_back(0xFFFFFFFFu);
    const uint32_t nr = (uint32_t)rules.size();
    if (kern.gsn > 64u) throw std::runtime_error("kvjit: more than 64 site-record groups in one kernel");
    std::ostringstream o;
    o << kern.decls;
    if (opt.stamps) o << "__device__ unsigned long long* kvj_stamps;\n";
    o << "__device__ const uint32_t " << name << "_rules[" << nr << "] = {";
    for (uint32_t q = 0; q < nr; q++) o << (q ? ", " : "") << u32(rules[q]);
    o << "};\n";
    const std::string lb = waves > 0 ? "KV_RWG, " + std::to_string(waves) : "KV_RWG";
    o << "extern \"C\" __global__ __launch_bounds__(" << lb << ") void " << name
      << "(const DevPS* __restrict__ Pp, const DevBatch* __restrict__ Bp, const Node* __restrict__ N, "
         "const Val* __restrict__ V, const uint8_t* __restrict__ S, DevOut O, uint32_t r0) {\n"
      << "  constexpr uint32_t FIN_ = " << u32(FIN) << ", ACT_ = " << u32(ACT) << ", ST_STORED_ = 0x7Eu;\n"
      << "  __shared__ unsigned long long s_stq[" << kernel_lds(nr) / 8 + (KV_RWAVES * kern.gsn + 1u) / 2u
      << "];\n  uint32_t* s_stw = (uint32_t*)s_stq;\n"
      << "  const DevPS& P = *Pp;\n  const DevBatch& B = *Bp;\n  const uint8_t* __restrict__ pstr = P.pstr;\n";
    o << "  const uint32_t nb_ = gridDim.x, x_ = blockIdx.x & 7u, per_ = nb_ >> 3, rem_ = nb_ & 7u;\n"
      << "  const uint32_t bx_ = x_ * per_ + (x_ < rem_ ? x_ : rem_) + (blockIdx.x >> 3);\n";
    o << "  const uint32_t r = r0 + bx_ * KV_RWG + threadIdx.x;\n"
      << "  const uint32_t n_res = B.n_res;\n"
      << "  const bool valid = r < n_res;\n"
      << "  const Res* __restrict__ R = B.res + (valid ? r : 0u);\n"
      << "  uint32_t root = ABSENT, rkind = KEY_NONE, rflags = 0u, rtup = 0u;\n"
      << "  if (valid) { root = ni(kv_gld(&R->root, 0)); rkind = kv_gld(&R->kind, 0); rflags = kv_gld(&R->flags, 0); rtup = kv_gld(&R->tup, 0); }\n"
      << "  Node rootn{0u, 0u, 0u, 0u};\n";
    o << "  const uint32_t* __restrict__ PC = B.pcol;\n"
        << "  const uint32_t ln_ = threadIdx.x & " << u32(KV_LANES - 1) << ", gw_ = (r >> 6) * KVC_W0;\n"
        << "  if (valid) rootn = " << col_macro("LD", 0, 0) << "(gw_);\n";
    o
      << "  const uint32_t* __restrict__ mtr_ = P.mtup + rtup;\n  const uint32_t ntup_ = B.n_tup;\n"
      << "  uint8_t* s_w = (uint8_t*)s_stw;\n"
      << "  uint32_t* const s_gc_ = s_stw + " << u32(kernel_lds(nr) / 4u) << ";\n"
      << (kern.gsn ? "  for (uint32_t t_ = threadIdx.x; t_ < " + u32(KV_RWAVES * kern.gsn) + "; t_ += KV_RWG) s_gc_[t_] = 0u;\n"
                : std::string())
      << "  kv_prefill_rows(s_stw, " << nr << "u, r - threadIdx.x, n_res);\n";
    auto stamp = [&](size_t k) {
      if (opt.stamps && k < kJitStamps)
        o << "  if (kvj_stamps && (threadIdx.x & 63u) == 0u) kvj_stamps[((size_t)blockIdx.x * KV_RWAVES + (threadIdx.x >> 6)) * "
          << kJitStamps << "u + " << k << "u] = __builtin_amdgcn_s_memtime();\n";
    };
    stamp(0);
    for (size_t bi = 0; bi < blocks.size(); bi++) {
      const uint32_t r0 = rows[bi].first, rn = rows[bi].second;
      const uint32_t p0 = kern.mt_kbase * 32u + r0, p1 = p0 + rn;
      o << "  {\n";
      std::string any = "0u";
      for (uint32_t w = p0 / 32u; w * 32u < p1; w++) {
        const uint32_t lo = std::max(p0, w * 32u) - w * 32u, hi = std::min(p1, w * 32u + 32u) - w * 32u;
        const uint32_t m = hi - lo == 32u ? 0xFFFFFFFFu : ((1u << (hi - lo)) - 1u) << lo;
        o << "  const uint32_t mw" << w << " = valid ? kv_gld(mtr_, (size_t)" << w << "u * ntup_) : 0u;\n";
        any += " | (mw" + std::to_string(w) + " & " + u32(m) + ")";
      }
      o << "  if (__ballot((" << any << ") != 0u) != 0ull) {\n" << blocks[bi] << "  }\n";
      o << "  }\n";
      stamp(bi + 1);
    }
    o << "  const uint32_t wg0_ = r - threadIdx.x;\n";
    if (kern.gsn)
      o << "#ifndef KVEMU\n  if ((KV_OFULL(O) & 2u) && !(KV_OFULL(O) & 4u) && (threadIdx.x & 63u) < " << u32(kern.gsn)
        << " && r - (threadIdx.x & 63u) < n_res)\n    O.gcnt[(size_t)(" << u32(kern.gs0)
        << " + (threadIdx.x & 63u)) * ((n_res + 63u) >> 6) + (r >> 6)] = s_gc_[(threadIdx.x & 63u) * KV_RWAVES + (threadIdx.x >> 6)];\n#endif\n";
    o << "  kv_end_flush(O, s_stw, " << nr << "u, " << name << "_rules, n_res, r, valid, "
         "(KV_OFULL(O) & 8u) && valid ? O.scope[r] : 0xFFFFFFFFu, (KV_OFULL(O) & 8u) && wg0_ < n_res ? O.scope[wg0_] : 0xFFFFFFFFu, "
         "P.n_rules);\n";
    stamp(std::min<size_t>(blocks.size() + 1, kJitStamps - 1));
    o << "}\n\n";
    kernels.push_back({name, o.str()});
    return rules;
  }

  void build_fac(JitImage* out) const {
    const uint32_t W = (uint32_t)(mt_bits.size() / 32u);
    out->fac_word.assign(4u * W, 0u);
    out->fac_bit.clear();
    out->fac_flist.clear();
    out->fac_rule = mt_bits;
    auto planes = [&](uint32_t mode, uint32_t first, uint32_t count) {
      std::vector<std::vector<uint32_t>> p;
      if (mode == 1) {
        for (uint32_t f = first; f < first + count; f++) p.push_back({f});
      } else if (mode == 2) {
        std::vector<uint32_t> all;
        for (uint32_t f = first; f < first + count; f++) all.push_back(f);
        p.push_back(all);
      } else {
        p.push_back({first});
      }
      return p;
    };
    uint32_t slot = 0;
    for (uint32_t w = 0; w < W; w++) {
      std::vector<std::vector<std::vector<uint32_t>>> mp(32), xp(32);
      uint32_t nm = 0, nx = 0, named = 0, cx = 0;
      for (uint32_t b = 0; b < 32u; b++) {
        const uint32_t ri = mt_bits[w * 32u + b];
        if (ri == 0xFFFFFFFFu) continue;
        if (name_dependent(ri)) {
          named |= 1u << b;
          continue;
        }
        const RuleRec& rr = ps.rules[ri];
        auto m = planes(rr.m_mode, rr.m_first, rr.m_count), x = planes(rr.x_mode, rr.x_first, rr.x_count);
        if (m.size() > KV_FAC_MAXP || x.size() > KV_FAC_MAXP) {
          cx |= 1u << b;
          continue;
        }
        nm = std::max<uint32_t>(nm, (uint32_t)m.size());
        nx = std::max<uint32_t>(nx, (uint32_t)x.size());
        mp[b] = std::move(m);
        xp[b] = std::move(x);
      }
      out->fac_word[4u * w] = slot;
      out->fac_word[4u * w + 1] = nm | nx << 8;
      out->fac_word[4u * w + 2] = named;
      out->fac_word[4u * w + 3] = cx;
      for (uint32_t p = 0; p < nm + nx; p++, slot++)
        for (uint32_t b = 0; b < 32u; b++) {
          const auto& pl = p < nm ? mp[b] : xp[b];
          const uint32_t k = p < nm ? p : p - nm;
          if (k < pl.size()) {
            out->fac_bit.push_back((uint32_t)out->fac_flist.size());
            out->fac_bit.push_back((uint32_t)pl[k].size() | KV_FAC_PRESENT);
            out->fac_flist.insert(out->fac_flist.end(), pl[k].begin(), pl[k].end());
          } else {
            out->fac_bit.push_back(0u);
            out->fac_bit.push_back(0u);
          }
        }
    }
    out->fac_slots = slot;
    if (out->fac_flist.empty()) out->fac_flist.push_back(0u);
    if (out->fac_bit.empty()) out->fac_bit.assign(2, 0u);
  }

  uint32_t rule_weight(uint32_t ri) {
    if (no_program(ps.rules[ri])) return 0;
    const RGen g = analyze(ri);
    uint32_t w = 2 + g.maxd;
    if (!g.loops.empty()) w += 4 * (g.max_level + 1);
    if (g.uses_anchor) w += 4;
    if (g.uses_keyglob) w += 3;
    return w;
  }

  std::vector<uint32_t> initial_blocks(const std::vector<uint32_t>& sorted, uint32_t a, uint32_t e) {
    if (opt.block_w) return initial_blocks_w(sorted, a, e, opt.block_w);
    std::vector<uint32_t> out = initial_blocks_w(sorted, a, e, 160u);
    if (out.size() >= 6) out = initial_blocks_w(sorted, a, e, 240u);
    return out;
  }
  std::vector<uint32_t> initial_blocks_w(const std::vector<uint32_t>& sorted, uint32_t a, uint32_t e, uint32_t budget) {
    std::vector<uint32_t> out;
    std::set<std::string> seen;
    uint32_t cur = 0, w = 0;
    for (uint32_t q = a; q < e; q++) {
      const uint32_t ri = sorted[q];
      const std::string& f = form_of(ri).text;
      const uint32_t rw = rule_weight(ri);
      if (cur > 0 && w + (seen.count(f) ? 0u : rw) > budget) {
        out.push_back(cur);
        cur = 0;
        w = 0;
        seen.clear();
      }
      cur++;
      if (!seen.count(f)) w += rw;
      if (!f.empty()) seen.insert(f);
    }
    if (cur) out.push_back(cur);
    return out;
  }
};

std::string rule_signature(const PolicySet& ps, uint32_t ri) {
  std::vector<std::string> expr(64);
  expr[0] = "R";
  std::string arr;
  std::vector<std::string> leaves;
  int nest = 0;
  for (uint32_t pc = ps.rules[ri].prog;; pc++) {
    const Inst& in = ps.prog[pc];
    const uint32_t op = in.op & 0xFF, d = (in.op >> 8) & 0xFF, aux = (in.op >> 16) & 0xFF;
    if (op == OP_DONE || d + 1 >= expr.size()) break;
    switch (op) {
      case OP_KEY:
      case OP_KEYV:
        expr[d + 1] = expr[d].empty() ? "" : expr[d] + ((aux & AUX_SCAN) ? "/k" : "/s") + std::to_string(in.a);
        break;
      case OP_LEAF:
        leaves.push_back(expr[d]);
        break;
      case OP_LOOP_BEGIN:
      case OP_EXIST_BEGIN:
        if (op == OP_LOOP_BEGIN && nest == 0 && arr.empty()) {
          arr = expr[d].empty() ? "?" : expr[d];
          expr[d + 1] = "E";
        } else {
          expr[d + 1].clear();
        }
        nest++;
        break;
      case OP_LOOP_END:
      case OP_EXIST_END:
        nest--;
        break;
      case OP_KEYGLOB:
      case OP_INDEX:
        expr[d + 1].clear();
        break;
      default:
        break;
    }
  }
  std::sort(leaves.begin(), leaves.end());
  std::string sig = (arr.empty() ? "~" : arr) + "|";
  for (auto& l : leaves) sig += l + ",";
  return sig;
}

std::string rule_kind_key(const PolicySet& ps, uint32_t ri) {
  const RuleRec& rr = ps.rules[ri];
  std::vector<std::string> ks;
  for (uint32_t f = rr.m_first; f < rr.m_first + rr.m_count; f++) {
    const MFilter& F = ps.filters[f];
    if (!(F.flags & MF_KINDS)) return "*";
    for (uint32_t i = F.kinds_first; i < F.kinds_first + F.kinds_count; i++) {
      const KindSpec& k = ps.kinds[i];
      if (k.form == 3) return "*";
      ks.push_back(std::to_string(k.kind));
    }
  }
  std::sort(ks.begin(), ks.end());
  ks.erase(std::unique(ks.begin(), ks.end()), ks.end());
  std::string key;
  for (auto& k : ks) key += k + ",";
  return key;
}

std::vector<uint32_t> rule_order(const PolicySet& ps) {
  std::vector<std::pair<std::string, uint32_t>> order;
  for (uint32_t ri = 0; ri < ps.rules.size(); ri++)
    order.push_back({!no_program(ps.rules[ri]) ? "0" + rule_kind_key(ps, ri) + "#" + rule_signature(ps, ri) : "1", ri});
  std::stable_sort(order.begin(), order.end());
  std::vector<uint32_t> sorted;
  for (auto& o : order) sorted.push_back(o.second);
  return sorted;
}

std::vector<JitKernelPlan> first_plan(Gen& g, const std::vector<uint32_t>& sorted, uint32_t chunk_rules) {
  const uint32_t n = (uint32_t)sorted.size();
  if (chunk_rules == 0 || chunk_rules > KV_KROWS) chunk_rules = KV_KROWS;
  uint32_t parts = (n + chunk_rules - 1) / chunk_rules;
  while (parts < n && Gen::lds_waves((n + parts - 1) / parts) < Gen::lds_waves(n / parts)) parts++;
  std::vector<JitKernelPlan> plan;
  for (uint32_t k = 0; k < parts; k++) {
    const uint32_t a = (uint32_t)((uint64_t)n * k / parts), e = (uint32_t)((uint64_t)n * (k + 1) / parts);
    std::vector<uint32_t> bl = g.initial_blocks(sorted, a, e);
    const int lds_waves = Gen::lds_waves(e - a);
    const int rule_waves = (int)std::max<uint32_t>(1u, (160u * 1024u) / std::max<uint32_t>(1u, (e - a) * 256u));
    plan.push_back({a, e - a, g.opt.has_waves ? g.opt.waves : std::min({8, lds_waves, rule_waves}), bl, true});
  }
  return plan;
}

void assemble_programs(const Gen& g, const std::string& prelude, const std::string& cdefs, JitImage* out) {
  const std::vector<std::pair<std::string, std::string>>& defs = g.helpers;
  std::unordered_map<std::string, size_t> def_index;
  for (size_t i = 0; i < defs.size(); i++) def_index[defs[i].first] = i;
  auto refs = [&](const std::string& text, std::vector<size_t>* out_ids) {
    static const char* prefixes[] = {"g_glob_", "g_atom_", "g_pred_", "g_blk_", "g_match_",
                                     "g_dleaf_", "q_glob_", "q_atom_", "q_pred_", "r_glob_", "r_atom_", "r_pred_"};
    for (const char* pf : prefixes) {
      const size_t pl = strlen(pf);
      for (size_t q = text.find(pf); q != std::string::npos; q = text.find(pf, q + pl)) {
        size_t e = q + pl;
        while (e < text.size() && isdigit((unsigned char)text[e])) e++;
        auto it = def_index.find(text.substr(q, e - q));
        if (it != def_index.end()) out_ids->push_back(it->second);
      }
    }
  };
  out->common = prelude;
  out->kernel_name.clear();
  out->kernel_src.clear();
  out->source = prelude + cdefs;
  for (const auto& d : defs) out->source += d.second;
  for (auto& k : g.kernels) {
    std::vector<char> used(defs.size(), 0);
    std::vector<size_t> stack;
    refs(k.second, &stack);
    while (!stack.empty()) {
      const size_t d = stack.back();
      stack.pop_back();
      if (used[d]) continue;
      used[d] = 1;
      refs(defs[d].second, &stack);
    }
    std::string prog;
    for (size_t d = 0; d < defs.size(); d++)
      if (used[d]) prog += defs[d].second;
    out->kernel_name.push_back(k.first);
    out->kernel_src.push_back(cdefs + prog + k.second);
    out->source += k.second;
  }
}

}

uint32_t jit_chunk_rules() {
  const char* ch = getenv("KVGPU_JIT_CHUNK");
  return ch && atoi(ch) > 0 ? std::min<uint32_t>((uint32_t)atoi(ch), KV_KROWS) : KV_KROWS;
}

void jit_generate(const PolicySet& ps, uint32_t chunk_rules, JitImage* out) {
  auto t0 = std::chrono::steady_clock::now();
  Gen g(ps);
  g.use_seed = out->col_use;
  const std::string prelude =
      g.opt.diag + kPrelude + std::string("\nusing namespace kv;\n\n") +
      "__device__ __noinline__ bool kv_dleaf_impl(const DevBatch& B, const Node* __restrict__ N, uint32_t dp, Node vn);\n\n";
  for (uint32_t ri = 0; ri < ps.rules.size(); ri++)
    if (!no_program(ps.rules[ri])) g.leaf_classes(ri);
  for (uint32_t ri = 0; ri < ps.rules.size(); ri++) g.match_fn(ri);
  out->chunks.clear();
  const uint32_t n = (uint32_t)ps.rules.size();
  const std::vector<uint32_t> sorted = rule_order(ps);
  if (out->plan.empty() && n) out->plan = first_plan(g, sorted, chunk_rules);
  for (const JitKernelPlan& kp : out->plan) {
    JitChunk kc;
    kc.name = "kvj_r" + std::to_string(kp.first) + "_" + std::to_string(kp.count) +
              (kp.blocks.size() > 1 ? "_b" + std::to_string(kp.blocks.size()) : "") + (kp.waves ? "" : "u");
    for (uint32_t q = kp.first; q < kp.first + kp.count; q++) kc.rules.push_back(sorted.at(q));
    std::vector<std::vector<uint32_t>> bl;
    uint32_t at = 0;
    for (uint32_t c : kp.blocks) {
      if (at + c > kp.count) break;
      bl.emplace_back(kc.rules.begin() + at, kc.rules.begin() + at + c);
      at += c;
    }
    if (at != kp.count) throw std::runtime_error("kvjit: kernel plan blocks do not cover its rules");
    kc.rules = g.group_kernel(kc.name, bl, kp.waves, kp.grouped);
    out->chunks.push_back(kc);
  }
  out->mtup_words = (uint32_t)(g.mt_bits.size() / 32u);
  if (out->mtup_words && !out->probe) g.build_fac(out);
  out->rec_compact.assign(n, 1);
  for (uint32_t ri = 0; ri < n; ri++) out->rec_compact[ri] = g.rec_slot[ri] ? 0 : 1;
  out->gs_desc = g.gs_desc;
  out->gs_mem = g.gs_mem;
  out->gs_members = g.gs_members;
  std::string cdefs;
  g.col_plan(out, &cdefs);

  out->memo_preds.clear();
  out->memo_words = 0;
  if (!g.mpreds.empty() && !out->probe) {
    g.ptab_kernel();
    out->memo_preds = g.mpreds;
    out->memo_words = (uint32_t)((g.mpreds.size() + 31) / 32);
    out->ptab_row = g.ptab_row_out();
  }
  assemble_programs(g, prelude, cdefs, out);
  out->gen_ms = std::chrono::duration<double, std::milli>(std::chrono::steady_clock::now() - t0).count();
}

}
```

kyverno_amd/csrc/kvkernel.hip:

```cpp
#include <hip/hip_runtime.h>
#include <stdint.h>

#include <algorithm>

#include "kvdev.h"

using namespace kv;

#define KV_RCHUNK 64

#include "kvdevfn.h"
#include "kvfac.h"
#include "kvcol.h"
#include "kvblocks.h"
#include "kvforeach.h"
#include "kvwalk.h"

extern "C" __global__ __launch_bounds__(KV_WG) __attribute__((amdgpu_waves_per_eu(4))) void kv_validate_kernel(const DevPS* __restrict__ Pp,
                                                                      const DevBatch* __restrict__ Bp, DevOut O,
                                                                      uint32_t rule_begin, uint32_t rule_end,
                                                                      uint32_t n_chunks, uint32_t rblocks) {
  __shared__ uint32_t s_cur[KV_MAXD][KV_WG];
  __shared__ uint32_t s_lfirst[KV_MAXL][KV_WG];
  __shared__ uint32_t s_llen[KV_MAXL][KV_WG];
// ... 621 lines not shown
    *(uint32_t*)(o + (size_t)k * (KV_RWG / 2) + 4u * j) = v;
  }
}

hipError_t launch_status_pack(const uint8_t* status, const uint8_t* sflag, uint32_t n_res, uint32_t n_rules,
                              const unsigned long long* cbase, uint32_t* ccnt, uint8_t* out, hipStream_t stream) {
  if (n_res == 0 || n_rules == 0) return hipSuccess;
  const uint32_t nwg = (n_res + KV_RWG - 1) / KV_RWG, nch = (nwg + KV_WG - 1) / KV_WG;
  for (uint32_t q0 = 0; q0 < n_rules; q0 += kMaxGridY) {
    hipLaunchKernelGGL(kv_status_pack_kernel, dim3(nch, std::min(kMaxGridY, n_rules - q0)), dim3(KV_WG), 0, stream,
                       status, sflag, cbase, ccnt, n_res, nwg, nch, out, q0);
    if (hipError_t e = hipGetLastError(); e != hipSuccess) return e;
  }
  return hipSuccess;
}


hipError_t launch_rec_compact(const uint8_t* status, const ErrRec8* err8, const ErrRec* errw, uint32_t n_res,
                              uint32_t n_rules, uint32_t* offs, unsigned long long* totals, unsigned long long* base,
                              ErrRec8* out8, ErrRec* outw, uint32_t* wide, int phase, const uint8_t* compact,
                              const uint32_t* order, unsigned long long* masks, const uint8_t* sflag,
                              hipStream_t stream) {
  if (n_res == 0 || n_rules == 0) return hipSuccess;
  const uint32_t tiles = (n_res + KV_WG - 1) / KV_WG;
  const uint32_t gx = std::max(1u, std::min(tiles, 65536u / n_rules));
  for (uint32_t q0 = 0; q0 < n_rules; q0 += kMaxGridY) {
    const dim3 grid(gx, std::min(kMaxGridY, n_rules - q0));
    if (phase == 0)
      hipLaunchKernelGGL(kv_rec_count_kernel, grid, dim3(KV_WG), 0, stream, status, n_res, tiles, offs, masks, sflag, q0);
    else
      hipLaunchKernelGGL(kv_rec_scatter_kernel, grid, dim3(KV_WG), 0, stream, status, err8, errw, n_res, tiles, offs,
                         base, out8, outw, wide, compact, order, masks, sflag, q0);
    if (hipError_t e = hipGetLastError(); e != hipSuccess) return e;
  }
  if (phase == 0) {
    hipLaunchKernelGGL(kv_rec_scan_kernel, dim3(n_rules), dim3(KV_WG), 0, stream, offs, tiles, totals);
    hipLaunchKernelGGL(kv_rec_base_kernel, dim3(1), dim3(KV_WG), 0, stream, totals, n_rules, base);
  }
  return hipGetLastError();
}

}

namespace kv {

__global__ __launch_bounds__(KV_WG) void kv_scope_count_kernel(const uint8_t* __restrict__ status,
                                                                const uint32_t* __restrict__ scope, uint32_t n_res,
                                                                uint32_t n_rules, uint32_t n_scopes,
                                                                unsigned long long* __restrict__ out) {
  extern __shared__ uint32_t s_cnt[];
  const uint32_t rule = blockIdx.x % n_rules;
  const uint32_t chunk = blockIdx.x / n_rules;
  const bool in_lds = n_scopes <= KV_SCOPE_LDS;
  if (in_lds)
    for (uint32_t q = threadIdx.x; q < n_scopes * KV_HIST; q += KV_WG) s_cnt[q] = 0;
  __syncthreads();
  const uint64_t row = (uint64_t)rule * n_res;
  const uint32_t base = chunk * KV_SCOPE_CHUNK;
  const uint32_t end = min(base + KV_SCOPE_CHUNK, n_res);
  for (uint32_t i = base + threadIdx.x * 4; i < end; i += KV_WG * 4) {
    uint32_t sc[4];
    uint32_t st[4];
    if (i + 4 <= end) {
      const uint4 s4 = *(const uint4*)(scope + i);
      sc[0] = s4.x; sc[1] = s4.y; sc[2] = s4.z; sc[3] = s4.w;
#pragma unroll
      for (int k = 0; k < 4; k++) st[k] = status[row + i + k];
    } else {
#pragma unroll
      for (int k = 0; k < 4; k++) {
        sc[k] = i + k < end ? scope[i + k] : 0xFFFFFFFFu;
        st[k] = i + k < end ? status[row + i + k] : 0;
      }
    }
#pragma unroll
    for (int k = 0; k < 4; k++) {
      if (sc[k] >= n_scopes || st[k] >= KV_HIST) continue;
      if (in_lds) atomicAdd(&s_cnt[sc[k] * KV_HIST + st[k]], 1u);
      else atomicAdd(&out[((uint64_t)sc[k] * n_rules + rule) * KV_HIST + st[k]], 1ull);
    }
  }
  if (!in_lds) return;
  __syncthreads();
  for (uint32_t q = threadIdx.x; q < n_scopes * KV_HIST; q += KV_WG) {
    const uint32_t v = s_cnt[q];
    if (v) atomicAdd(&out[((uint64_t)(q / KV_HIST) * n_rules + rule) * KV_HIST + q % KV_HIST], (unsigned long long)v);
  }
}

hipError_t launch_scope_counts(const uint8_t* status, const uint32_t* scope, uint32_t n_res, uint32_t n_rules,
                               uint32_t n_scopes, unsigned long long* out, hipStream_t stream) {
  if (n_res == 0 || n_rules == 0 || n_scopes == 0) return hipSuccess;
  const uint32_t chunks = (n_res + KV_SCOPE_CHUNK - 1) / KV_SCOPE_CHUNK;
  const size_t shm = n_scopes <= KV_SCOPE_LDS ? (size_t)n_scopes * KV_HIST * sizeof(uint32_t) : 0;
  hipLaunchKernelGGL(kv_scope_count_kernel, dim3(chunks * n_rules), dim3(KV_WG), shm, stream, status, scope, n_res,
                     n_rules, n_scopes, out);
  return hipGetLastError();
}

__global__ __launch_bounds__(KV_WG) void kv_scope_totals_kernel(const unsigned long long* __restrict__ sc,
                                                                uint32_t n_scopes, uint32_t n,
                                                                unsigned long long* __restrict__ counts) {
  const uint32_t i = blockIdx.x * KV_WG + threadIdx.x;
  if (i >= n) return;
  unsigned long long t = 0ull;
  for (uint32_t s = 0; s < n_scopes; s++) t += sc[(size_t)s * n + i];
  counts[i] = t;
}

hipError_t launch_scope_totals(const unsigned long long* scounts, uint32_t n_scopes, uint32_t n_rules,
                               unsigned long long* counts, hipStream_t stream) {
  const uint32_t n = n_rules * (uint32_t)KV_HIST;
  if (n == 0) return hipSuccess;
  hipLaunchKernelGGL(kv_scope_totals_kernel, dim3((n + KV_WG - 1) / KV_WG), dim3(KV_WG), 0, stream, scounts, n_scopes,
                     n, counts);
  return hipGetLastError();
}

__global__ __launch_bounds__(KV_WG) void kv_expand_rows_kernel(const uint64_t* __restrict__ tcells,
                                                               const uint64_t* __restrict__ rmask,
                                                               const uint64_t* __restrict__ rwide,
                                                               const uint32_t* __restrict__ roff,
                                                               const Val* __restrict__ vals, uint64_t n_rows,
                                                               Node* __restrict__ nodes) {
  const uint64_t row = (uint64_t)blockIdx.x * (KV_WG / KV_LANES) + threadIdx.x / KV_LANES;
  if (row >= n_rows) return;
  const uint32_t lane = threadIdx.x & (KV_LANES - 1);
  const uint64_t m = rmask[row], below = (1ull << lane) - 1ull;
  Node v{0u, 0u, 0u, 0u};
  if ((m >> lane) & 1ull) {
    const uint64_t w = rwide[row];
    const uint64_t* u = tcells + roff[row] + (uint32_t)__popcll(m & below) + (uint32_t)__popcll(w & below);
    const uint64_t x = u[0];
    if ((w >> lane) & 1ull) {
      const uint64_t y = u[1];
      v = Node{(uint32_t)x, (uint32_t)(x >> 32), (uint32_t)y, (uint32_t)(y >> 32)};
    } else {
      v = cell_widen((uint32_t)x, (uint32_t)(x >> 32), row, vals);
    }
  }
  nodes[row * KV_LANES + lane] = v;
}

hipError_t launch_expand_rows(const uint64_t* tcells, const uint64_t* rmask, const uint64_t* rwide, const uint32_t* roff,
                              const Val* vals, uint64_t n_rows, Node* nodes, hipStream_t stream) {
  if (n_rows == 0) return hipSuccess;
  const uint64_t blocks = (n_rows + KV_WG / KV_LANES - 1) / (KV_WG / KV_LANES);
  if (blocks > 0x7FFFFFFFull) return hipErrorInvalidValue;
  hipLaunchKernelGGL(kv_expand_rows_kernel, dim3((uint32_t)blocks), dim3(KV_WG), 0, stream, tcells, rmask, rwide, roff,
                     vals, n_rows, nodes);
  return hipGetLastError();
}

__global__ __launch_bounds__(KV_WG) void kv_pcol_rows_kernel(const DevBatch* __restrict__ Bp,
                                                             const ColDesc* __restrict__ cols,
                                                             const ColFam* __restrict__ fams) {
  const uint32_t r = blockIdx.x * KV_WG + threadIdx.x, f = 1u + blockIdx.y;
  uint32_t v = col_rows(*Bp, cols, fams, f, r);
#pragma unroll
  for (int m = 1; m < (int)KV_LANES; m <<= 1) v = max(v, (uint32_t)__shfl_xor((int)v, m, (int)KV_LANES));
  if ((threadIdx.x & (KV_LANES - 1)) == 0) fams[f].erow[r >> 6] = v;
}

__global__ __launch_bounds__(1024) void kv_pcol_scan_kernel(const ColFam* __restrict__ fams, uint32_t n_groups) {
  __shared__ uint32_t s_sum[1024];
  uint32_t* __restrict__ e = fams[1u + blockIdx.x].erow;
  const uint32_t per = (n_groups + 1023u) / 1024u, a = threadIdx.x * per, b = min(a + per, n_groups);
  uint32_t t = 0;
  for (uint32_t i = a; i < b; i++) t += e[i];
  s_sum[threadIdx.x] = t;
  __syncthreads();
  for (uint32_t o = 1; o < 1024u; o <<= 1) {
    const uint32_t x = threadIdx.x >= o ? s_sum[threadIdx.x - o] : 0u;
    __syncthreads();
    s_sum[threadIdx.x] += x;
    __syncthreads();
  }
  uint32_t run = s_sum[threadIdx.x] - t;
  for (uint32_t i = a; i < b; i++) {
    const uint32_t c = e[i];
    e[i] = run;
    run += c;
  }
  if (threadIdx.x == 1023u) e[n_groups] = s_sum[1023];
}

__global__ __launch_bounds__(KV_WG) void kv_pcol_build_kernel(const DevBatch* __restrict__ Bp,
                                                              const ColDesc* __restrict__ cols,
                                                              const ColFam* __restrict__ fams, uint32_t c0,
                                                              uint32_t elem, uint32_t* __restrict__ pool) {
  const uint32_t r = blockIdx.x * KV_WG + threadIdx.x, c = c0 + blockIdx.y;
  if (elem) col_build_elem(*Bp, cols, fams, c, r, pool);
  else col_build_root(*Bp, cols, fams, c, r, pool);
}

hipError_t launch_pcol_rows(const DevBatch* B, const ColDesc* cols, const ColFam* fams, uint32_t n_fam,
                            uint32_t n_groups, hipStream_t stream) {
  if (n_fam < 2 || n_groups == 0) return hipSuccess;
  hipLaunchKernelGGL(kv_pcol_rows_kernel, dim3(n_groups * KV_LANES / KV_WG, n_fam - 1), dim3(KV_WG), 0, stream, B, cols,
                     fams);
  if (hipError_t e = hipGetLastError()) return e;
  hipLaunchKernelGGL(kv_pcol_scan_kernel, dim3(n_fam - 1), dim3(1024), 0, stream, fams, n_groups);
  return hipGetLastError();
}

hipError_t launch_pcol_build(const DevBatch* B, const ColDesc* cols, const ColFam* fams, uint32_t c0, uint32_t n,
                             uint32_t n_groups, bool elem, uint32_t* pool, hipStream_t stream) {
  if (n == 0 || n_groups == 0) return hipSuccess;
  if (n > 65535u) return hipErrorInvalidValue;
  hipLaunchKernelGGL(kv_pcol_build_kernel, dim3(n_groups * KV_LANES / KV_WG, n), dim3(KV_WG), 0, stream, B, cols, fams,
                     c0, elem ? 1u : 0u, pool);
  return hipGetLastError();
}

}
```

Baseline: 327.6 billion evals/s.

## Add nested array column families and emit JIT loops over precomputed path columns

```diff
diff --git a/kyverno_amd/csrc/kvapi.cpp b/kyverno_amd/csrc/kvapi.cpp
--- a/kyverno_amd/csrc/kvapi.cpp
+++ b/kyverno_amd/csrc/kvapi.cpp
@@ -192,8 +192,11 @@
   HIPCHK(hipMemset(d->perow.p, 0, d->perow.n));
   std::vector<ColFam> fams(nf);
   uint32_t n_wide = 0, n_narrow = 0;
+  bool nested = false;
   for (uint32_t f = 0; f < nf; f++) {
     fams[f].arr_col = J.fam_arr[f];
+    fams[f].parent = J.fam_parent.at(f);
+    nested = nested || fams[f].parent != 0;
     fams[f].ncols = J.fam_ncols[f];
     fams[f].nw = J.fam_nw.at(f);
     fams[f].nb = J.fam_nb.at(f);
@@ -209,7 +212,7 @@
   const ColDesc* cd = (const ColDesc*)d->pcold.p;
   std::vector<uint32_t> erow;
   if (nf > 1) {
-    HIPCHK(launch_pcol_rows(Bd, cd, (const ColFam*)d->pfam.p, nf, groups, nullptr));
+    HIPCHK(launch_pcol_rows(Bd, cd, (const ColFam*)d->pfam.p, nf, nested, groups, nullptr));
     erow.resize((size_t)(nf - 1) * (groups + 1));
     HIPCHK(hipMemcpy(erow.data(), d->perow.p, erow.size() * sizeof(uint32_t), hipMemcpyDeviceToHost));
   }
@@ -226,9 +229,10 @@
   d->pcol.alloc(std::max<uint64_t>(words, 1) * sizeof(uint32_t), device);
   uint32_t* pool = (uint32_t*)d->pcol.p;
   if (words > root_words) HIPCHK(hipMemset(pool + root_words, 0, (words - root_words) * sizeof(uint32_t)));
-  HIPCHK(launch_pcol_build(Bd, cd, (const ColFam*)d->pfam.p, 0, j0, groups, false, pool, nullptr));
-  HIPCHK(launch_pcol_build(Bd, cd, (const ColFam*)d->pfam.p, j0, (uint32_t)J.cols.size() - j0, groups, true, pool,
-                           nullptr));
+  HIPCHK(launch_pcol_build(Bd, cd, (const ColFam*)d->pfam.p, 0, j0, groups, 0u, pool, nullptr));
+  for (uint32_t level = 1; level <= (nested ? 2u : 1u); level++)
+    HIPCHK(launch_pcol_build(Bd, cd, (const ColFam*)d->pfam.p, j0, (uint32_t)J.cols.size() - j0, groups, level, pool,
+                             nullptr));
   HIPCHK(hipStreamSynchronize(nullptr));
   d->view.pcol = pool;
   d->pcol_ms = std::chrono::duration<double, std::milli>(std::chrono::steady_clock::now() - t0).count();
diff --git a/kyverno_amd/csrc/kvcol.h b/kyverno_amd/csrc/kvcol.h
--- a/kyverno_amd/csrc/kvcol.h
+++ b/kyverno_amd/csrc/kvcol.h
@@ -67,10 +67,31 @@
   return Node{w[0], w[1], pool[row + (size_t)(3u * F.nw + d.bpos) * KV_LANES + lane], w[2]};
 }
 
+KV_FN Node col_root_arr(const uint32_t* __restrict__ pool, const ColDesc* cols, const ColFam* fams, const ColFam& F,
+                        uint32_t r) {
+  return col_get(pool, (uint64_t)(r >> 6) * col_row_words(fams[0]), fams[0], cols[F.arr_col], r & (KV_LANES - 1));
+}
+KV_FN bool col_is_arr(const Node& a) { return a.kt != 0u && node_type(a.kt) == NT_ARR; }
+
 KV_FN uint32_t col_rows(const DevBatch& B, const ColDesc* cols, const ColFam* fams, uint32_t f, uint32_t r) {
   if (r >= B.n_res) return 0u;
   uint32_t idx;
   const Node n = col_walk(B.nodes, ni(B.res[r].root), cols[fams[f].arr_col], &idx);
+  return idx != ABSENT && node_type(n.kt) == NT_ARR ? n.b : 0u;
+}
+
+KV_FN Node col_nested_parent(const DevBatch& B, const ColDesc* cols, const ColFam* fams, uint32_t f, uint32_t r) {
+  const Node z{0u, 0u, 0u, 0u};
+  if (r >= B.n_res) return z;
+  uint32_t idx;
+  const Node a = col_walk(B.nodes, ni(B.res[r].root), cols[fams[fams[f].parent].arr_col], &idx);
+  return idx != ABSENT && node_type(a.kt) == NT_ARR ? a : z;
+}
+KV_FN uint32_t col_rows_nested(const DevBatch& B, const ColDesc* cols, const ColFam* fams, uint32_t f, const Node& a,
+                               uint32_t i) {
+  if (i >= a.b) return 0u;
+  uint32_t idx;
+  const Node n = col_walk(B.nodes, ni(a.a + i), cols[fams[f].arr_col], &idx);
   return idx != ABSENT && node_type(n.kt) == NT_ARR ? n.b : 0u;
 }
 
@@ -91,16 +112,45 @@
   col_put(pool, (uint64_t)(r >> 6) * col_row_words(fams[0]), fams[0], d, r & (KV_LANES - 1), cell, idx);
 }
 
+KV_FN uint32_t col_build_elem_at(const DevBatch& B, const ColDesc* cols, const ColFam* fams, uint32_t c, uint32_t r, uint32_t i,
+                             uint32_t arr_c, uint32_t* __restrict__ pool) {
+  const ColDesc& d = cols[c];
+  const ColFam& F = fams[d.fam];
+  const Node a = col_root_arr(pool, cols, fams, F, r);
+  if (!col_is_arr(a) || i >= a.b) return 0u;
+  uint32_t idx;
+  const Node n = col_walk(B.nodes, ni(a.a + i), d, &idx);
+  col_put(pool, (uint64_t)a.c + (uint64_t)i * col_row_words(F), F, d, r & (KV_LANES - 1), col_cell(n, idx, arr_c), idx);
+  return idx != ABSENT && node_type(n.kt) == NT_ARR ? n.b : 0u;
+}
+KV_FN uint32_t col_elems(const ColDesc* cols, const ColFam* fams, uint32_t c, uint32_t r, const uint32_t* __restrict__ pool) {
+  const Node a = col_root_arr(pool, cols, fams, fams[cols[c].fam], r);
+  return col_is_arr(a) ? a.b : 0u;
+}
+KV_FN uint32_t col_nested_off(const ColFam& N, uint32_t g, uint32_t run) {
+  return (uint32_t)(col_fam_off(N) + (uint64_t)(N.erow[g] + run) * col_row_words(N));
+}
+
 KV_FN void col_build_elem(const DevBatch& B, const ColDesc* cols, const ColFam* fams, uint32_t c, uint32_t r,
                           uint32_t* __restrict__ pool) {
+  for (uint32_t i = 0, n = col_elems(cols, fams, c, r, pool); i < n; i++) col_build_elem_at(B, cols, fams, c, r, i, 0u, pool);
+}
+
+KV_FN void col_build_nested(const DevBatch& B, const ColDesc* cols, const ColFam* fams, uint32_t c, uint32_t r,
+                            uint32_t* __restrict__ pool) {
   const ColDesc& d = cols[c];
   const ColFam& F = fams[d.fam];
+  const ColFam& P = fams[F.parent];
   const uint32_t lane = r & (KV_LANES - 1);
-  const Node a = col_get(pool, (uint64_t)(r >> 6) * col_row_words(fams[0]), fams[0], cols[F.arr_col], lane);
-  if (node_type(a.kt) != NT_ARR || a.kt == 0u) return;
+  const Node a = col_root_arr(pool, cols, fams, P, r);
+  if (!col_is_arr(a)) return;
   for (uint32_t i = 0; i < a.b; i++) {
-    uint32_t idx;
-    const Node n = col_walk(B.nodes, ni(a.a + i), d, &idx);
-    col_put(pool, (uint64_t)a.c + (uint64_t)i * col_row_words(F), F, d, lane, col_cell(n, idx, 0u), idx);
+    const Node e = col_get(pool, (uint64_t)a.c + (uint64_t)i * col_row_words(P), P, cols[F.arr_col], lane);
+    if (!col_is_arr(e)) continue;
+    for (uint32_t k = 0; k < e.b; k++) {
+      uint32_t idx;
+      const Node n = col_walk(B.nodes, ni(e.a + k), d, &idx);
+      col_put(pool, (uint64_t)e.c + (uint64_t)k * col_row_words(F), F, d, lane, col_cell(n, idx, 0u), idx);
+    }
   }
 }
diff --git a/kyverno_amd/csrc/kvdev.h b/kyverno_amd/csrc/kvdev.h
--- a/kyverno_amd/csrc/kvdev.h
+++ b/kyverno_amd/csrc/kvdev.h
@@ -56,9 +56,9 @@
 hipError_t launch_expand_rows(const uint64_t* tcells, const uint64_t* rmask, const uint64_t* rwide, const uint32_t* roff,
                               const Val* vals, uint64_t n_rows, Node* nodes, hipStream_t stream);
 
-hipError_t launch_pcol_rows(const DevBatch* B, const ColDesc* cols, const ColFam* fams, uint32_t n_fam,
+hipError_t launch_pcol_rows(const DevBatch* B, const ColDesc* cols, const ColFam* fams, uint32_t n_fam, bool nested,
                             uint32_t n_groups, hipStream_t stream);
 hipError_t launch_pcol_build(const DevBatch* B, const ColDesc* cols, const ColFam* fams, uint32_t c0, uint32_t n,
-                             uint32_t n_groups, bool elem, uint32_t* pool, hipStream_t stream);
+                             uint32_t n_groups, uint32_t level, uint32_t* pool, hipStream_t stream);
 
 }
diff --git a/kyverno_amd/csrc/kvdevtypes.h b/kyverno_amd/csrc/kvdevtypes.h
--- a/kyverno_amd/csrc/kvdevtypes.h
+++ b/kyverno_amd/csrc/kvdevtypes.h
@@ -105,6 +105,7 @@
 };
 struct ColFam {
   uint32_t arr_col, ncols;
+  uint32_t parent;
   uint32_t nw, nb, nn;
   uint32_t off_lo, off_hi;
   uint32_t* erow;
diff --git a/kyverno_amd/csrc/kvjit.hpp b/kyverno_amd/csrc/kvjit.hpp
--- a/kyverno_amd/csrc/kvjit.hpp
+++ b/kyverno_amd/csrc/kvjit.hpp
@@ -19,6 +19,7 @@
   int waves;
   std::vector<uint32_t> blocks;
   bool grouped = false;
+  bool colloops = false;
 };
 
 struct JitImage {
@@ -38,7 +39,7 @@
   std::vector<uint32_t> gs_desc, gs_mem;
   uint32_t gs_members = 0;
   std::vector<kv::ColDesc> cols;
-  std::vector<uint32_t> fam_arr, fam_ncols;
+  std::vector<uint32_t> fam_arr, fam_parent, fam_ncols;
   std::vector<uint32_t> fam_nw, fam_nb, fam_nn;
   std::map<std::string, uint32_t> col_use;
   bool probe = false;
diff --git a/kyverno_amd/csrc/kvjitbuild.cpp b/kyverno_amd/csrc/kvjitbuild.cpp
--- a/kyverno_amd/csrc/kvjitbuild.cpp
+++ b/kyverno_amd/csrc/kvjitbuild.cpp
@@ -292,7 +292,9 @@
     changed = true;
     JitKernelPlan np = kp;
     const size_t big = (size_t)(std::max_element(np.blocks.begin(), np.blocks.end()) - np.blocks.begin());
-    if (kp.grouped) {
+    if (kp.colloops) {
+      np.colloops = false;
+    } else if (kp.grouped) {
       np.grouped = false;
     } else if (v.calls && v.fits) {
       np.waves = 0;
@@ -427,7 +429,7 @@
     if (line.rfind("kernel ", 0) != 0) continue;
     std::istringstream ls(line.substr(7));
     JitKernelPlan kp{0, 0, 0, {}};
-    ls >> kp.first >> kp.count >> kp.waves >> kp.grouped;
+    ls >> kp.first >> kp.count >> kp.waves >> kp.grouped >> kp.colloops;
     uint32_t sum = 0;
     for (uint32_t b; ls >> b; sum += b) kp.blocks.push_back(b);
     if (sum != kp.count || kp.blocks.empty()) return false;
@@ -444,7 +446,7 @@
   std::string t;
   for (const JitKernelPlan& kp : img.plan) {
     t += "kernel " + std::to_string(kp.first) + " " + std::to_string(kp.count) + " " + std::to_string(kp.waves) + " " +
-         (kp.grouped ? "1" : "0");
+         (kp.grouped ? "1" : "0") + " " + (kp.colloops ? "1" : "0");
     for (uint32_t b : kp.blocks) t += " " + std::to_string(b);
     t += "\n";
   }
@@ -459,22 +461,27 @@
 }
 
 static void jit_group_regions(const PolicySet& ps, uint32_t chunk, JitImage* img) {
-  for (JitKernelPlan& kp : img->plan) kp.grouped = true;
-  jit_generate(ps, chunk, img);
-  jit_compile(img);
-  bool back = false;
-  for (size_t k = 0; k < img->plan.size(); k++) {
-    RegVerdict v;
-    if (!reg_verdict(*img, program_of(*img, img->chunks[k].name), img->plan[k].waves, &v))
-      throw std::runtime_error("kvjit: no kernel descriptor for " + img->chunks[k].name);
-    if (!v.ships()) {
-      img->plan[k].grouped = false;
-      back = true;
-    }
-  }
-  if (!back) return;
-  jit_generate(ps, chunk, img);
-  jit_compile(img);
+  static const bool kSteps[4][2] = {{true, true}, {true, false}, {false, true}, {false, false}};
+  std::vector<int> step(img->plan.size(), 0);
+  for (int round = 0; round < 4; round++) {
+    for (size_t k = 0; k < img->plan.size(); k++) {
+      img->plan[k].grouped = kSteps[step[k]][0];
+      img->plan[k].colloops = kSteps[step[k]][1];
+    }
+    jit_generate(ps, chunk, img);
+    jit_compile(img);
+    bool back = false;
+    for (size_t k = 0; k < img->plan.size(); k++) {
+      RegVerdict v;
+      if (!reg_verdict(*img, program_of(*img, img->chunks[k].name), img->plan[k].waves, &v))
+        throw std::runtime_error("kvjit: no kernel descriptor for " + img->chunks[k].name);
+      if (!v.ships() && step[k] < 3) {
+        step[k]++;
+        back = true;
+      }
+    }
+    if (!back) return;
+  }
 }
 
 void jit_build(const PolicySet& ps, JitImage* img) {
@@ -486,7 +493,7 @@
     const std::string pkey = jit_plan_key(*img);
     const bool stored = jit_load_plan(pkey, img);
     if (!stored) {
-      for (JitKernelPlan& kp : img->plan) kp.grouped = false;
+      for (JitKernelPlan& kp : img->plan) kp.grouped = kp.colloops = false;
       jit_refine_blocks(ps, chunk, img);
     }
     jit_generate(ps, chunk, img);
diff --git a/kyverno_amd/csrc/kvjitgen.cpp b/kyverno_amd/csrc/kvjitgen.cpp
--- a/kyverno_amd/csrc/kvjitgen.cpp
+++ b/kyverno_amd/csrc/kvjitgen.cpp
@@ -3,6 +3,7 @@
 #include <cstdio>
 #include <cstdlib>
 #include <cstring>
+#include <list>
 #include <map>
 #include <set>
 #include <sstream>
@@ -43,13 +44,15 @@
 constexpr uint32_t kGslotMembers = 22u;
 
 struct GenOpts {
-  bool narrow, stamps, has_waves;
+  bool narrow, colloops, stamps, has_waves;
   int waves;
   uint32_t block_w;
   std::string diag;
   GenOpts() {
     const char* e = getenv("KVGPU_JIT_NARROW");
     narrow = !(e && e[0] == '0');
+    e = getenv("KVGPU_JIT_COLLOOPS");
+    colloops = !(e && e[0] == '0');
     stamps = getenv("KVGPU_JIT_STAMPS") != nullptr;
     e = getenv("KVGPU_JIT_WAVES");
     has_waves = e != nullptr;
@@ -65,6 +68,7 @@
 struct Gen {
   struct Fam {
     std::string arr;
+    uint32_t parent = 0, arr_j = 0;
     std::map<std::string, uint32_t> idx;
     std::vector<std::vector<uint32_t>> steps;
     std::vector<uint32_t> use;
@@ -103,6 +107,7 @@
     uint32_t gs0 = 0, gsn = 0;
     std::string decls;
     bool grouped = false;
+    bool colloops = false;
   };
 
   explicit Gen(const PolicySet& p) : ps(p), rec_slot(p.rules.size(), 0) {
@@ -152,20 +157,27 @@
     F.use.push_back(0u);
     return j;
   }
-  uint32_t family(const std::string& arr) {
+  uint32_t family(uint32_t parent, const std::string& rel) {
+    if (parent && fams.at(parent).parent) return kNoCol;
+    const std::string arr = parent ? fams[parent].arr + "[]" + rel : rel;
     auto it = fam_of.find(arr);
     if (it != fam_of.end()) return it->second;
-    if (col_of(0, arr) == kNoCol) return kNoCol;
+    const uint32_t j = col_of(parent, rel);
+    if (j == kNoCol) return kNoCol;
     const uint32_t f = (uint32_t)fams.size();
     fams.emplace_back();
     fams.back().arr = arr;
+    fams.back().parent = parent;
+    fams.back().arr_j = j;
     col_of(f, "");
     fam_of.emplace(arr, f);
     return f;
   }
+  uint32_t family(const std::string& arr) { return family(0, arr); }
   void col_plan(JitImage* out, std::string* defs) const {
     out->cols.clear();
     out->fam_arr.clear();
+    out->fam_parent.clear();
     out->fam_ncols.clear();
     out->fam_nw.clear();
     out->fam_nb.clear();
@@ -175,9 +187,14 @@
     d << "#define KVC_LO_ROW(n, w) kv_leaf_word(P, N, n, w)\n"
       << "#define KVC_LW_ROW(n, w) kv_leaf_gather(P, n, w)\n"
       << "#define KVC_LA_ROW(n, w) kv_leaf_fix(P.ptab, P.n_vals, N, (n).a, (n).b, false, w)\n";
+    std::vector<uint32_t> col0(fams.size(), 0u);
+    for (uint32_t f = 1; f < fams.size(); f++) col0[f] = col0[f - 1] + (uint32_t)fams[f - 1].steps.size();
+    std::set<std::pair<uint32_t, uint32_t>> arrs;
+    for (uint32_t f = 1; f < fams.size(); f++) arrs.insert({fams[f].parent, fams[f].arr_j});
     for (uint32_t f = 0; f < fams.size(); f++) {
       const Fam& F = fams[f];
-      out->fam_arr.push_back(f ? fams[0].idx.at(F.arr) : 0u);
+      out->fam_arr.push_back(f ? col0[F.parent] + F.arr_j : 0u);
+      out->fam_parent.push_back(F.parent);
       out->fam_ncols.push_back((uint32_t)F.steps.size());
       std::vector<uint32_t> use(F.steps.size(), 0u);
       for (const auto& kv : F.idx) {
@@ -185,7 +202,7 @@
         uint32_t u = F.use[kv.second];
         auto it = use_seed.find(key);
         if (it != use_seed.end()) u |= it->second;
-        if (f == 0 && fam_of.count(kv.first)) u |= CU_WIDE | CU_B;
+        if (arrs.count({f, kv.second})) u |= CU_WIDE | CU_B;
         use[kv.second] = u;
         out->col_use[key] = u;
       }
@@ -859,7 +876,16 @@
     uint32_t n = 0;
     int fam = -1;
     std::string troot, cell0;
-    std::string flush(bool grouped) {
+    static std::string joined(const std::vector<std::string>& xs) {
+      std::string s;
+      for (size_t i = 0; i < xs.size(); i += 8) {
+        s += "#ifndef KVEMU\n  asm volatile(\"\" ::";
+        for (size_t k = i; k < xs.size() && k < i + 8; k++) s += (k > i ? ", \"v\"(" : " \"v\"(") + xs[k] + ")";
+        s += ");\n#endif\n";
+      }
+      return s;
+    }
+    std::string flush(bool grouped, const std::vector<std::string>* join = nullptr) {
       std::string s;
       if (!grouped) {
         for (; oflushed < order.size(); oflushed++) {
@@ -876,6 +902,12 @@
       }
       oflushed = order.size();
       for (; cflushed < cells.size(); cflushed++) s += cells[cflushed];
+      if (join) {
+        std::vector<std::string> xs = *join;
+        for (const auto& kv : vars)
+          if (kv.second.fam >= 0) xs.push_back(kv.second.node + ".kt");
+        s += joined(xs);
+      }
       if (wflushed == words.size()) return s;
       std::vector<std::string> nodes;
       std::string fix;
@@ -887,6 +919,11 @@
         if (std::find(nodes.begin(), nodes.end(), x.hv.node) == nodes.end()) nodes.push_back(x.hv.node);
         fix += "    if (node_type(" + x.hv.node + ".kt) == NT_ARR) " + x.var + " = " +
                (col ? col_macro("LA", (uint32_t)x.hv.fam, x.hv.j) : std::string("KVC_LA_ROW")) + args;
+      }
+      if (join) {
+        std::vector<std::string> xs;
+        for (size_t i = wflushed; i < words.size(); i++) xs.push_back(words[i].var);
+        s += joined(xs);
       }
       wflushed = words.size();
       s += "  if (__ballot(";
@@ -999,8 +1036,25 @@
     }
   };
 
-  void emit_region(Block& B, RGen& g, const Region& R, std::ostream& w) {
+  struct ColLoop {
+    uint32_t body_pc = 0, end_pc = 0, fam = 0;
+    std::string troot;
+    HoistTable T;
+    std::ostringstream body;
+    std::ostream* outer = nullptr;
+  };
+
+  void emit_region(Block& B, RGen& g, const Region& R, std::ostream& w0) {
     const std::string& s = g.s;
+    std::list<ColLoop> cloops;
+    std::ostream* wcur = &w0;
+    auto cloop_of = [&](const std::string& ex) -> ColLoop* {
+      for (auto it = cloops.rbegin(); it != cloops.rend(); ++it) {
+        const size_t n = it->troot.size();
+        if (ex.compare(0, n, it->troot) == 0 && (ex.size() == n || ex[n] == '/')) return &*it;
+      }
+      return nullptr;
+    };
     auto C = [&](uint32_t d) { return "c" + std::to_string(d) + s; };
     auto L = [&](uint32_t pc) { return "R" + std::to_string(g.ri) + "_L" + std::to_string(pc); };
     auto jump = [&](uint32_t t, bool err = false) -> std::string {
@@ -1057,7 +1111,7 @@
     auto known = [&](uint32_t d) {
       if (d >= g.expr.size() || g.expr[d].empty()) return false;
       const std::string& ex = g.expr[d];
-      return ex[0] == 'R' || (R.T && ex.compare(0, R.troot.size(), R.troot) == 0);
+      return ex[0] == 'R' || (R.T && ex.compare(0, R.troot.size(), R.troot) == 0) || cloop_of(ex);
     };
     auto IDX = [&](uint32_t d) {
       if (d < g.csrc.size())
@@ -1075,6 +1129,7 @@
       const std::string& ex = g.expr[d];
       if (ex[0] == 'R') return &B.global;
       if (R.T && ex.compare(0, R.troot.size(), R.troot) == 0) return R.T;
+      if (ColLoop* cl = cloop_of(ex)) return &cl->T;
       return nullptr;
     };
     auto absent_or = [&](uint32_t d, const char* cmp) {
@@ -1110,13 +1165,26 @@
              s + "); " + jump(body) + " }\n";
     };
 
+    auto close_cloop = [&](uint32_t pc, const std::string& lv) {
+      if (cloops.empty() || cloops.back().end_pc != pc) return;
+      ColLoop& cl = cloops.back();
+      const std::string& p = cl.T.prefix;
+      const std::vector<std::string> join{p + "n.kt"};
+      *cl.outer << L(cl.body_pc) << ":;\n  const uint32_t " << p << "e = " << p << "c + li" << lv << s << " * KVC_W" << cl.fam
+                << ";\n  const Node " << p << "n = " << col_macro("LD", cl.fam, 0) << "(" << p << "e);\n"
+                << cl.T.flush(B.kern.grouped, &join) << cl.body.str() << "  }\n";
+      wcur = cl.outer;
+      cloops.pop_back();
+    };
+
     for (uint32_t pc = R.rb; pc < R.re; pc++) {
       const Inst& in = ps.prog[pc];
       const uint32_t op = in.op & 0xFF, d = (in.op >> 8) & 0xFF, aux = (in.op >> 16) & 0xFF;
       const std::string cd = C(d), cn = C(d + 1);
       const uint32_t lv = aux & 3;
       const std::string L_lv = std::to_string(lv);
-      w << L(pc) << ":;\n";
+      std::ostream& w = *wcur;
+      if (cloops.empty() || cloops.back().body_pc != pc) w << L(pc) << ":;\n";
       switch (op) {
         case OP_MAPCHK:
           w << "  if (" << absent_or(d, "!= NT_MAP") << ") " << raise(E_TYPE_MAP, in.a, in.c) << "\n";
@@ -1217,6 +1285,37 @@
           [[fallthrough]];
         case OP_EXIST_BEGIN:
           if (G && op == OP_EXIST_BEGIN) throw std::runtime_error("kvjit: EXIST in a rule group");
+          {
+            uint32_t f = kNoCol;
+            HoistTable* AT = opt.colloops && B.kern.colloops && known(d) ? table_for(d) : nullptr;
+            if (AT && AT->fam >= 0 && g.hv[d].fam == AT->fam && g.hv[d].j != kNoCol)
+              f = family((uint32_t)AT->fam, AT->fam == 0 ? g.expr[d] : g.expr[d].substr(AT->troot.size()));
+            if (f != kNoCol) {
+              const std::string an = NODE(d, CU_WIDE | CU_B);
+              set_unknown(d + 1);
+              cloops.emplace_back();
+              ColLoop& cl = cloops.back();
+              cl.body_pc = pc + 1;
+              cl.end_pc = in.a;
+              cl.fam = f;
+              cl.troot = "P" + std::to_string(pc);
+              cl.T.prefix = "p" + std::to_string(pc) + "_";
+              cl.T.fam = (int)f;
+              cl.T.troot = cl.troot;
+              cl.T.cell0 = cl.T.prefix + "e";
+              cl.outer = wcur;
+              g.expr[d + 1] = cl.troot;
+              g.hv[d + 1] = HVar{cn, cl.T.prefix + "n", (int)f, 0u};
+              w << "  { uint32_t " << cl.T.prefix << "c;\n  { const Node an_ = " << an << "; lf" << L_lv << s << " = an_.a; ll" << L_lv
+                << s << " = node_type(an_.kt) == NT_ARR ? an_.b : 0u; li" << L_lv << s << " = 0u; " << cl.T.prefix
+                << "c = an_.c;\n    if (ll" << L_lv << s << " == 0u) ";
+              if (op == OP_LOOP_BEGIN) w << jump(in.a + 1);
+              else w << raise(E_EXIST_FAIL, in.b, in.c);
+              w << "\n    " << cn << " = ni(an_.a); }\n";
+              wcur = &cl.body;
+              break;
+            }
+          }
           set_unknown(d + 1);
           w << "  { const Node an_ = " << NODE(d, CU_WIDE | CU_B) << "; lf" << L_lv << s << " = an_.a; ll" << L_lv << s << " = an_.b; li"
             << L_lv << s << " = 0u;\n    if (an_.b == 0u) ";
@@ -1230,12 +1329,14 @@
               << jump(in.c, true) << " }\n";
           w << next_elem(L_lv, cn, in.a + 1);
           set_unknown(d + 1);
+          close_cloop(pc, L_lv);
           break;
         case OP_EXIST_END:
           if (G) throw std::runtime_error("kvjit: EXIST in a rule group");
           w << "  if (!" << kindof << ") " << jump(pc + 1) << "\n  " << ek << " = 0u;\n"
             << next_elem(L_lv, cn, in.a + 1) << "  " << raise(E_EXIST_FAIL, in.b, in.c) << "\n";
           set_unknown(d + 1);
+          close_cloop(pc, L_lv);
           break;
         case OP_ALT_BEGIN:
           if (G) throw std::runtime_error("kvjit: anyPattern in a rule group");
@@ -1263,6 +1364,7 @@
           break;
       }
     }
+    if (!cloops.empty()) throw std::runtime_error("kvjit: a loop of rule " + std::to_string(g.ri) + " does not end in its region");
   }
 
   RGen analyze(uint32_t ri) {
@@ -1878,7 +1980,7 @@
     return (int)std::max<uint32_t>(1u, (160u * 1024u) / std::max(b, g) * KV_RWAVES / 4u);
   }
   std::vector<uint32_t> group_kernel(const std::string& name, const std::vector<std::vector<uint32_t>>& chs, int waves,
-                                     bool grouped) {
+                                     bool grouped, bool colloops) {
     std::vector<std::string> blocks;
     std::vector<std::pair<uint32_t, uint32_t>> rows;
     std::vector<uint32_t> rules;
@@ -1889,6 +1991,7 @@
     kern.mt_kbase = (uint32_t)(mt_bits.size() / 32u);
     kern.gs0 = (uint32_t)(gs_desc.size() / 4u);
     kern.grouped = grouped;
+    kern.colloops = colloops;
     for (const auto& c : chs) {
       std::vector<uint32_t> ord;
       rows.push_back({(uint32_t)rules.size(), (uint32_t)c.size()});
@@ -2156,7 +2259,7 @@
     std::vector<uint32_t> bl = g.initial_blocks(sorted, a, e);
     const int lds_waves = Gen::lds_waves(e - a);
     const int rule_waves = (int)std::max<uint32_t>(1u, (160u * 1024u) / std::max<uint32_t>(1u, (e - a) * 256u));
-    plan.push_back({a, e - a, g.opt.has_waves ? g.opt.waves : std::min({8, lds_waves, rule_waves}), bl, true});
+    plan.push_back({a, e - a, g.opt.has_waves ? g.opt.waves : std::min({8, lds_waves, rule_waves}), bl, true, true});
   }
   return plan;
 }
@@ -2237,7 +2340,7 @@
       at += c;
     }
     if (at != kp.count) throw std::runtime_error("kvjit: kernel plan blocks do not cover its rules");
-    kc.rules = g.group_kernel(kc.name, bl, kp.waves, kp.grouped);
+    kc.rules = g.group_kernel(kc.name, bl, kp.waves, kp.grouped, kp.colloops);
     out->chunks.push_back(kc);
   }
   out->mtup_words = (uint32_t)(g.mt_bits.size() / 32u);
diff --git a/kyverno_amd/csrc/kvkernel.hip b/kyverno_amd/csrc/kvkernel.hip
--- a/kyverno_amd/csrc/kvkernel.hip
+++ b/kyverno_amd/csrc/kvkernel.hip
@@ -797,13 +797,25 @@
   return hipGetLastError();
 }
 
+__device__ __forceinline__ uint32_t kv_wave_max(uint32_t v) {
+#pragma unroll
+  for (int m = 1; m < (int)KV_LANES; m <<= 1) v = max(v, (uint32_t)__shfl_xor((int)v, m, (int)KV_LANES));
+  return v;
+}
+
 __global__ __launch_bounds__(KV_WG) void kv_pcol_rows_kernel(const DevBatch* __restrict__ Bp,
                                                              const ColDesc* __restrict__ cols,
-                                                             const ColFam* __restrict__ fams) {
+                                                             const ColFam* __restrict__ fams, uint32_t nested) {
   const uint32_t r = blockIdx.x * KV_WG + threadIdx.x, f = 1u + blockIdx.y;
-  uint32_t v = col_rows(*Bp, cols, fams, f, r);
-#pragma unroll
-  for (int m = 1; m < (int)KV_LANES; m <<= 1) v = max(v, (uint32_t)__shfl_xor((int)v, m, (int)KV_LANES));
+  if ((fams[f].parent != 0u) != (nested != 0u)) return;
+  uint32_t v = 0u;
+  if (!nested) {
+    v = kv_wave_max(col_rows(*Bp, cols, fams, f, r));
+  } else {
+    const uint32_t n = fams[fams[f].parent].erow[r >> 6];
+    const Node a = col_nested_parent(*Bp, cols, fams, f, r);
+    for (uint32_t i = 0; i < n; i++) v += kv_wave_max(col_rows_nested(*Bp, cols, fams, f, a, i));
+  }
   if ((threadIdx.x & (KV_LANES - 1)) == 0) fams[f].erow[r >> 6] = v;
 }
 
@@ -833,29 +845,46 @@
 __global__ __launch_bounds__(KV_WG) void kv_pcol_build_kernel(const DevBatch* __restrict__ Bp,
                                                               const ColDesc* __restrict__ cols,
                                                               const ColFam* __restrict__ fams, uint32_t c0,
-                                                              uint32_t elem, uint32_t* __restrict__ pool) {
+                                                              uint32_t level, uint32_t* __restrict__ pool) {
   const uint32_t r = blockIdx.x * KV_WG + threadIdx.x, c = c0 + blockIdx.y;
-  if (elem) col_build_elem(*Bp, cols, fams, c, r, pool);
-  else col_build_root(*Bp, cols, fams, c, r, pool);
-}
-
-hipError_t launch_pcol_rows(const DevBatch* B, const ColDesc* cols, const ColFam* fams, uint32_t n_fam,
+  const ColDesc& d = cols[c];
+  if (level == 0u) {
+    col_build_root(*Bp, cols, fams, c, r, pool);
+    return;
+  }
+  if ((fams[d.fam].parent != 0u) != (level == 2u)) return;
+  if (level == 2u) {
+    col_build_nested(*Bp, cols, fams, c, r, pool);
+  } else if (!d.arr_fam) {
+    col_build_elem(*Bp, cols, fams, c, r, pool);
+  } else {
+    const ColFam& nf = fams[d.arr_fam];
+    const uint32_t n = kv_wave_max(col_elems(cols, fams, c, r, pool));
+    for (uint32_t i = 0, run = 0; i < n; i++) {
+      run += kv_wave_max(col_build_elem_at(*Bp, cols, fams, c, r, i, col_nested_off(nf, r >> 6, run), pool));
+    }
+  }
+}
+
+hipError_t launch_pcol_rows(const DevBatch* B, const ColDesc* cols, const ColFam* fams, uint32_t n_fam, bool nested,
                             uint32_t n_groups, hipStream_t stream) {
   if (n_fam < 2 || n_groups == 0) return hipSuccess;
-  hipLaunchKernelGGL(kv_pcol_rows_kernel, dim3(n_groups * KV_LANES / KV_WG, n_fam - 1), dim3(KV_WG), 0, stream, B, cols,
-                     fams);
-  if (hipError_t e = hipGetLastError()) return e;
+  for (uint32_t lv = 0; lv < (nested ? 2u : 1u); lv++) {
+    hipLaunchKernelGGL(kv_pcol_rows_kernel, dim3(n_groups * KV_LANES / KV_WG, n_fam - 1), dim3(KV_WG), 0, stream, B, cols,
+                       fams, lv);
+    if (hipError_t e = hipGetLastError()) return e;
+  }
   hipLaunchKernelGGL(kv_pcol_scan_kernel, dim3(n_fam - 1), dim3(1024), 0, stream, fams, n_groups);
   return hipGetLastError();
 }
 
 hipError_t launch_pcol_build(const DevBatch* B, const ColDesc* cols, const ColFam* fams, uint32_t c0, uint32_t n,
-                             uint32_t n_groups, bool elem, uint32_t* pool, hipStream_t stream) {
+                             uint32_t n_groups, uint32_t level, uint32_t* pool, hipStream_t stream) {
   if (n == 0 || n_groups == 0) return hipSuccess;
   if (n > 65535u) return hipErrorInvalidValue;
   hipLaunchKernelGGL(kv_pcol_build_kernel, dim3(n_groups * KV_LANES / KV_WG, n), dim3(KV_WG), 0, stream, B, cols, fams,
-                     c0, elem ? 1u : 0u, pool);
-  return hipGetLastError();
-}
-
-}
+                     c0, level, pool);
+  return hipGetLastError();
+}
+
+}
```

Result: faster. 346.0 billion evals/s (median of 6 runs) (+5.6%).
